# maksimt/rri_nmf

Measured on AMD Instinct MI355X. Metric: RRI sweeps/sec and achieved HBM GB/s on dense X (n x d, rank k), higher is better.
Workload: dtype f64

## Files before the change

### include/rri_hip.h

```cpp
#ifndef RRI_HIP_H
#define RRI_HIP_H

#include <stdint.h>
#include <stddef.h>

#ifdef __cplusplus
extern "C" {
#endif

#define RRI_ABI_VERSION 1
#define RRI_GRAM_SLICES 8
#define RRI_MAX_K 1024

typedef struct rri_ctx rri_ctx;
typedef struct rri_comm rri_comm;
#define RRI_COMM_ID_BYTES 128

typedef int32_t rri_status;
enum {
    RRI_OK = 0,
    RRI_PAUSED = 1,
    RRI_ERR_INVALID = -1,
    RRI_ERR_HIP = -2,
    RRI_ERR_UNSUPPORTED = -3,
// ... 69 lines not shown
rri_status rri_residual_update(rri_ctx* ctx, const double* a, const double* b, const double* a2, const double* b2,
                               const double* trow, const double* wcol, double* y_out, double* z_out);
rri_status rri_get_residual(rri_ctx* ctx, void* host, int64_t ld, int32_t host_dtype);

rri_status rri_project_W_rows(rri_ctx* ctx, double s, const double* s_vec);
rri_status rri_objective(rri_ctx* ctx, double* out);
rri_status rri_argmax_rows(rri_ctx* ctx, int32_t* out_host);
rri_status rri_masked_rmse(rri_ctx* ctx, const int64_t* ij, const double* vals, int64_t count,
                           double clip_lo, double clip_hi, double* out);
rri_status rri_snapshot(rri_ctx* ctx);
rri_status rri_rollback(rri_ctx* ctx);

rri_status rri_X_times(rri_ctx* ctx, const double* B, int32_t m, double* out);
rri_status rri_Xt_times(rri_ctx* ctx, const double* Q, int32_t m, double* out);
rri_status rri_range_finder(rri_ctx* ctx, const double* Q0, int32_t m, int32_t n_iter, int32_t transpose, double* Q_out,
                            double* B_out);
rri_status rri_sparse_range_finder(rri_ctx* ctx, const double* Q0, int32_t m, int32_t n_iter, int32_t transpose, double* Q_out,
                                   double* B_out);

rri_status rri_column_positive_counts(rri_ctx* ctx, double* df_out);
rri_status rri_scale_X(rri_ctx* ctx, const double* col_scale, int32_t normalize_rows);
rri_status rri_csr_column_positive_counts(rri_ctx* ctx, double* df_out);
rri_status rri_csr_scale_X(rri_ctx* ctx, const double* col_scale, int32_t normalize_rows, int64_t* zero_rows_out);

rri_status rri_comm_unique_id(uint8_t* id_out );
rri_status rri_comm_create(rri_comm** out, const uint8_t* id, int32_t rank, int32_t world, int32_t device);
typedef int32_t (*rri_allreduce_fn)(void* user, double* buf, int64_t count);
typedef int32_t (*rri_allgather_fn)(void* user, const double* send, int64_t count, double* recv);
typedef int32_t (*rri_broadcast_fn)(void* user, double* buf, int64_t count, int32_t root);
rri_status rri_comm_create_host(rri_comm** out, int32_t rank, int32_t world, rri_allreduce_fn allreduce,
                                rri_allgather_fn allgather, rri_broadcast_fn broadcast, void* user);
rri_status rri_comm_destroy(rri_comm* comm);
rri_status rri_attach_comm(rri_ctx* ctx, rri_comm* comm, int64_t row_offset, int64_t n_global);
rri_status rri_comm_broadcast(rri_ctx* ctx, double* host, int64_t count, int32_t root);
rri_status rri_comm_allreduce_sum(rri_ctx* ctx, double* host, int64_t count);
rri_status rri_comm_stats(rri_ctx* ctx, int32_t* rank, int32_t* world, int64_t* allreduce_calls);

rri_status rri_reduce_buffer(rri_ctx* ctx, void** dev_ptr, int64_t* n_elems);
rri_status rri_bind_reduce_buffer(rri_ctx* ctx, void* dev_ptr, int64_t n_elems);
rri_status rri_topic_reduce_local(rri_ctx* ctx, int32_t t);
rri_status rri_reduce_read(rri_ctx* ctx, double* out, int64_t count);
rri_status rri_reduce_write(rri_ctx* ctx, const double* in, int64_t count);
rri_status rri_topic_finish(rri_ctx* ctx, int32_t t);
rri_status rri_topic_finish_w(rri_ctx* ctx, int32_t t);
rri_status rri_resid_row_argmax(rri_ctx* ctx, double* value, int64_t* local_row);
rri_status rri_reset_row(rri_ctx* ctx, int64_t local_row, double* row_out_host);
rri_status rri_poll(rri_ctx* ctx);
rri_status rri_objective_parts(rri_ctx* ctx, double out[3]);

rri_status rri_timing_enable(rri_ctx* ctx, int32_t on);
rri_status rri_timing_read(rri_ctx* ctx, int32_t kernel_id, int64_t* launches, double* total_ms);
rri_status rri_synchronize(rri_ctx* ctx);
rri_status rri_onchip_info(rri_ctx* ctx, int32_t* eligible, int64_t* launches);
#define RRI_LAYOUT_FIELDS 19
rri_status rri_layout_info(rri_ctx* ctx, int64_t* out, int32_t n);
rri_status rri_onchip_fallbacks(rri_ctx* ctx, int64_t* fallbacks);
rri_status rri_debug_xcc(rri_ctx* ctx, int32_t* out, int32_t count);
rri_status rri_sweep_until(rri_ctx* ctx, int32_t n_sweeps, double obj_prev, double stop_scale, double* obj_hist,
                           int32_t* sweeps_done);
rri_status rri_bench_rank1_update(rri_ctx* ctx, int32_t reps, double* avg_ms);
rri_status rri_bench_stream_copy(rri_ctx* ctx, int32_t reps, double* avg_ms);

#ifdef __cplusplus
}
#endif
#endif
```

### rri_nmf_amd/_capi.py

```python
import ctypes as C
import os

_PKG = os.path.dirname(os.path.abspath(__file__))
LIB_PATH = os.environ.get('RRI_HIP_LIB', os.path.join(_PKG, 'lib', 'librri_hip.so'))

RRI_GRAM_SLICES = 8
RRI_LAYOUT_FIELDS = 19
RRI_MAX_K = 1024
RRI_OK, RRI_PAUSED = 0, 1
RRI_ERR_INVALID, RRI_ERR_HIP, RRI_ERR_UNSUPPORTED = -1, -2, -3
RRI_ERR_UNBOUNDED, RRI_ERR_W_COL_ZERO, RRI_ERR_NOT_IMPLEMENTED, RRI_ERR_COMM = -4, -5, -6, -7
RRI_COMM_ID_BYTES = 128
RRI_F32, RRI_F64, RRI_F16 = 0, 1, 2
RRI_UNWEIGHTED, RRI_WEIGHTED_DENSE, RRI_WEIGHTED_SPARSE, RRI_UNWEIGHTED_RESIDUAL, RRI_UNWEIGHTED_SPARSE = 0, 1, 2, 3, 4
RESET_NONE, RESET_MAX_RESID_DOCUMENT, RESET_RANDOM = 0, 1, 2
EVENT_NONE, EVENT_RESET_T, EVENT_RESET_W = 0, 1, 2
ABI_VERSION = 1


class Params(C.Structure):
    _fields_ = [('fix_W', C.c_int32), ('fix_T', C.c_int32), ('project_T_each_iter', C.c_int32),
                ('has_t_row_sum', C.c_int32), ('has_w_row_sum', C.c_int32), ('reset_method', C.c_int32),
                ('resets_left', C.c_int32), ('reserved0', C.c_int32),
                ('t_row_sum', C.c_double), ('w_row_sum', C.c_double),
                ('reg_w_l1', C.c_double), ('reg_w_l2', C.c_double), ('reg_t_l1', C.c_double),
                ('reg_t_l2', C.c_double), ('eps_div', C.c_double)]


class Event(C.Structure):
    _fields_ = [('kind', C.c_int32), ('topic', C.c_int32), ('sweep', C.c_int32), ('resume_topic', C.c_int32)]


_P = C.c_void_p
_I32, _I64, _D = C.c_int32, C.c_int64, C.c_double
ALLREDUCE_FN = C.CFUNCTYPE(C.c_int32, C.c_void_p, C.POINTER(C.c_double), C.c_int64)
ALLGATHER_FN = C.CFUNCTYPE(C.c_int32, C.c_void_p, C.POINTER(C.c_double), C.c_int64, C.POINTER(C.c_double))
BROADCAST_FN = C.CFUNCTYPE(C.c_int32, C.c_void_p, C.POINTER(C.c_double), C.c_int64, C.c_int32)
PROTOTYPES = {
    'rri_abi_version': (C.c_uint32, []),
    'rri_create': (_I32, [C.POINTER(_P), _I64, _I64, _I32, _I32, _I32, _I32, _P]),
    'rri_destroy': (_I32, [_P]),
    'rri_last_error': (C.c_char_p, [_P]),
    'rri_upload_X': (_I32, [_P, _P, _I64, _I32]),
    'rri_upload_mask': (_I32, [_P, _P, _I64, _I32]),
    'rri_bind_X_device': (_I32, [_P, _P, _I64]),
    'rri_storage_error': (_I32, [_P, C.POINTER(_D)]),
    'rri_bind_mask_device': (_I32, [_P, _P, _I64]),
    'rri_upload_X_csr': (_I32, [_P, C.POINTER(_I64), C.POINTER(_I32), _P, _I64, _I32]),
    'rri_upload_mask_csr_pattern': (_I32, [_P, C.POINTER(_I64), C.POINTER(_I32), _P, _I64, _I32]),
    'rri_upload_observed_csr': (_I32, [_P, C.POINTER(_I64), C.POINTER(_I32), _P, _I64, _I32]),
    'rri_set_W': (_I32, [_P, _P, _I64, _I32]),
    'rri_set_T': (_I32, [_P, _P, _I64, _I32]),
    'rri_get_W': (_I32, [_P, _P, _I64, _I32]),
    'rri_get_T': (_I32, [_P, _P, _I64, _I32]),
    'rri_set_params': (_I32, [_P, C.POINTER(Params)]),
    'rri_sweep': (_I32, [_P, _I32, C.POINTER(_I32)]),
    'rri_resume': (_I32, [_P, C.POINTER(_I32)]),
    'rri_pending_event': (_I32, [_P, C.POINTER(Event)]),
    'rri_apply_reset_max_resid': (_I32, [_P, _I32, C.POINTER(_I64)]),
    'rri_apply_reset_vectors': (_I32, [_P, _I32, C.POINTER(_D), C.POINTER(_D)]),
# ... 113 lines not shown
```

### rri_nmf_amd/csrc/rri_hip.hip

```cpp
#include <hip/hip_runtime.h>
#include <dlfcn.h>
#include <rccl/rccl.h>

#include <algorithm>
#include <atomic>
#include <chrono>
#include <cstdarg>
#include <cstdio>
#include <mutex>
#include <cstdlib>
#include <cstring>
#include <string>
#include <utility>
#include <vector>

#include "rri_hip.h"
#include "rri_kernels.hpp"
#include "rri_wrri_kernels.hpp"
#include "rri_sparse_kernels.hpp"
#include "rri_onchip_kernels.hpp"

using namespace rri;

namespace {
// ... 39 lines not shown
        a.AllReduce = (decltype(a.AllReduce))dlsym(from, "ncclAllReduce");
        a.AllGather = (decltype(a.AllGather))dlsym(from, "ncclAllGather");
        a.Broadcast = (decltype(a.Broadcast))dlsym(from, "ncclBroadcast");
        a.GetErrorString = (decltype(a.GetErrorString))dlsym(from, "ncclGetErrorString");
        a.CommAbort = (decltype(a.CommAbort))dlsym(from, "ncclCommAbort");
        return a.GetUniqueId && a.CommInitRank && a.CommDestroy && a.AllReduce && a.AllGather && a.Broadcast &&
               a.GetErrorString;
    };
    if (const char* e = getenv("RRI_RCCL_LIB")) {
        h = dlopen(e, RTLD_NOW | RTLD_GLOBAL);
        if (h && resolve(h)) { a.ok = true; return a; }
        a.err = std::string("RRI_RCCL_LIB=") + e + " could not be used";
        return a;
    }
    if (resolve(RTLD_DEFAULT)) { a.ok = true; return a; }
    for (const char* name : {"librccl.so.1", "librccl.so"}) {
        h = dlopen(name, RTLD_NOW | RTLD_GLOBAL);
        if (h && resolve(h)) { a.ok = true; return a; }
    }
    a.err = "RCCL not found (no ncclAllReduce in the process, no librccl.so.1)";
    return a;
}
RcclApi& rccl_api() {
    static RcclApi api = load_rccl();
    return api;
}
}

struct rri_comm {
    int rank = 0, world = 1, device = 0;
    ncclComm_t nccl = nullptr;
    rri_allreduce_fn h_allreduce = nullptr;
    rri_allgather_fn h_allgather = nullptr;
    rri_broadcast_fn h_broadcast = nullptr;
    void* user = nullptr;
    std::vector<double> hbuf, hbuf2;
    long n_allreduce = 0;
    bool aborted = false;
};

constexpr double PASS_CACHE_MB = 256.0;

struct rri_switches {
    bool onchip = true;
    bool onchip_obj = true;
    bool wsweep = true;
    bool obj_direct = false;
    bool wmcorr_cols = true;
    bool wnw_mask = true;
    int pass_rot = -1;
    int rot_cal = 1;
    bool rot_debug = false;
    bool mask_bits = true;
    double pass_cache_mb = PASS_CACHE_MB;
};

struct rri_ctx {
    i64 n = 0, d = 0, LD = 0;
    int k = 0, dtype = RRI_F32, weighted = 0, device = 0;
    size_t es = 4;
    double store_err[2] = {0.0, 0.0};
    int VN = 4, PW = 1024;
    hipStream_t stream = nullptr;
    bool own_stream = false;
    rri_switches sw;

    void *X = nullptr, *M = nullptr, *E = nullptr;
    i64 ldx = 0, ldm = 0;
    bool own_X = false, own_M = false;
    double *W = nullptr, *T = nullptr, *Wprev = nullptr, *Tprev = nullptr;
    double *Ypart = nullptr, *Zpart = nullptr, *red = nullptr, *xraw = nullptr, *Ttpart = nullptr;
    unsigned* Mbits = nullptr;
    i64 ldb = 0;
    double* Qt = nullptr;
    bool q_valid = false;
    int rot_x = 0, rot_r = 0;
    bool rot_done = false;
    int keep_q = -1;
    bool gfull_valid = false;
    double *Gfull = nullptr, *Wsweep0 = nullptr, *wsum_part = nullptr, *wsums = nullptr;
    double *Y2part = nullptr, *Z2part = nullptr, *dtv = nullptr, *dwv = nullptr, *wold = nullptr, *zeros = nullptr;
    i64 ldw = 0;
    int nsplit = 4;
    bool own_red = false;
    i64 red_elems = 0;
    bool sparse = false;
    i64 nnz = 0;
    int sp_max_row = 0, kp = 8;
    i64* sp_rowptr = nullptr;
    int* sp_col = nullptr;
    void *sp_x = nullptr, *sp_e = nullptr;
    double* sp_Tt = nullptr;
    struct SpCopy {
        int nblk = 1, bw = 1, lps = 64, nwork = 0;
        i64 nseg = 0, gdim = 0, count = 0;
        i64* segptr = nullptr;
        unsigned short* idx = nullptr;
        void* val = nullptr;
        int* perm = nullptr;
        SpWork* work = nullptr;
    } sp[2];
    bool sparse_x = false;
    SpWork* spx_work = nullptr;
    double* rowhat = nullptr;
    double* Cpart = nullptr;
    double* N2part = nullptr;
    unsigned* Mcols = nullptr;
    bool nw_mask = false;
    bool mcols_tried = false;
    double mask_density = 1.0;
    int cpart_rows = 0;
    bool wcorr = false;
    int wcorr_topic = 0, wcorr_nrb = 0;
    bool resid_fresh = false;
    bool dt_pending = false;
    bool explicit_resid = false;
    bool dw_pending = false;
    int dw_topic = 0;
    double* told = nullptr;
    double *Gpart = nullptr, *tpart = nullptr, *rowobj = nullptr, *rowpos = nullptr, *normpart = nullptr;
    double *dtmp = nullptr;
    double* objbuf = nullptr;
    i64* itmp = nullptr;
    i64* tpart_idx = nullptr;
    double *resetT = nullptr, *resetW = nullptr;
    DevState* st = nullptr;

    int npanels = 1, rpb = 1, nrb = 1, nwb = 1, ntb = 1;
    int gpart_n = 1;
    int ttpart_n = 0;
    int xy_rows = 0;
    int xy_stride = 1;
    int ntb32 = 1;
    int tpart_n = 1;

    rri_params prm{};
    bool have_params = false, have_X = false, have_W = false, have_T = false, have_M = false;


    bool carry_valid = false;
    int carry_topic = -1;
    double* XYpart = nullptr;
    int xy_run = -1;
    bool xy_valid = false, x_sq_valid = false;
    bool obj_track_pending = false, obj_track_valid = false;
    double obj_track_value = 0.0;
    struct { bool active = false; double prev = 0.0, scale = 0.0; int n = 0; double* out = nullptr; } until;
    double *objhist = nullptr, *objdec = nullptr;
    double x_sq = 0.0;
    bool pending_wcheck = false;
    int pending_wcheck_topic = -1;

    bool paused = false;
    int run_total = 0;
    Cursor resume_at{0, 0, 0};
    bool resume_done = false;
    rri_event pending{RRI_EVENT_NONE, -1, 0, 0};

    bool resid_valid = false;
    bool skip_row_finish = false;
    int nwb256 = 1;

    rri_comm* comm = nullptr;
    i64 row_offset = 0, n_global = 0;
    double* ctail = nullptr;
    double* cand = nullptr;
    rri_status comm_status = RRI_OK;

    int n_cu = 0;
    double *mkZ = nullptr, *mkG = nullptr, *mkP = nullptr, *mkX = nullptr, *mkT = nullptr, *objE = nullptr;
    unsigned* mkbar = nullptr;
    long onchip_launches = 0;
    double *Wsafe = nullptr, *Tsafe = nullptr;
    bool onchip_in_flight = false;
    bool onchip_off = false;
    long long onchip_off_until = 0;
    bool onchip_saved_skip = false;
    long onchip_fallbacks = 0;

    int timing = 0;
    long timing_seq[4] = {0, 0, 0, 0};
    std::vector<TimedLaunch> timed[4];
    std::vector<hipEvent_t> event_pool;
// ... 140 lines not shown
    hipEvent_t e = nullptr;
    (void)hipEventCreate(&e);
    return e;
}
struct TimedScope {
    rri_ctx* c;
    int id;
    TimedLaunch tl{nullptr, nullptr};
    bool on;
    TimedScope(rri_ctx* c_, int id_)
        : c(c_), id(id_),
          on(c_->timing > 0 && (c_->timing_seq[id_]++ % c_->timing) == 0 && c_->timed[id_].size() < 400000) {
        if (on) {
            tl.a = get_event(c);
            tl.b = get_event(c);
            (void)hipEventRecord(tl.a, c->stream);
        }
    }
    ~TimedScope() {
        if (on) {
            (void)hipEventRecord(tl.b, c->stream);
            c->timed[id].push_back(tl);
        }
    }
};

size_t dtype_size(int dt) { return dt == RRI_F32 ? 4 : dt == RRI_F64 ? 8 : dt == RRI_F16 ? 2 : 0; }

void f16_unreachable(rri_ctx* c) {
    if (c->comm_status == RRI_OK) {
        c->comm_status = RRI_ERR_UNSUPPORTED;
        c->err = "this operation rewrites X or needs a mask, a residual or a CSR store: not available on an RRI_F16 handle";
    }
}

template <typename SX>
struct LaunchX {
    typedef SX Elem;
    static constexpr bool RO = std::is_same<SX, _Float16>::value;
    static size_t pass_shmem(const rri_ctx* c, int upd) {
        return ((5 + upd) * (size_t)c->rpb + 4 * 8 * 72) * sizeof(double);
    }
    struct Upd {
        const double *a = nullptr, *b = nullptr, *a2 = nullptr, *b2 = nullptr, *b2sub = nullptr;
    };
    static int stream_whole(const rri_ctx* c) {
        return (double)c->n * (double)c->LD * (double)c->es > 192.0e6 ? 0 : -1;
    }
    template <bool DO_Y, bool DO_Z, int UPD, int U, bool NT, bool RS>
    static void pass_k(rri_ctx* c, void* Xp, i64 ldp, const double* trow, const double* wc, const Upd& u, const TgramJob& job,
                       int keep) {
        const int ncols = (int)std::min<i64>(ldp, c->LD);
        typedef typename std::conditional<(UPD > 0), SX, const SX>::type XT;
        hipLaunchKernelGGL((k_pass<SX, DO_Y, DO_Z, UPD, U, NT, RS>), dim3(c->npanels * c->nrb + job.nblocks), dim3(256),
                           pass_shmem(c, UPD), c->stream, (XT*)Xp, ldp, (int)c->n, ncols, trow, wc, c->Ypart,
                           c->Zpart, c->LD, c->rpb, c->npanels, u.a, u.b, u.a2, u.b2, u.b2sub, (const DevState*)c->st, job,
                           ((ro_pass_interleaved(c) || UPD > 0) ? c->nrb : 0) |
                               ((c->sw.pass_rot >= 0 ? c->sw.pass_rot : (UPD > 0 ? c->rot_r : c->rot_x)) << 27),
                           keep);
    }
    template <bool DO_Y, bool DO_Z, int UPD>
    static void pass_cfg(rri_ctx* c, void* Xp, i64 ldp, const double* trow, const double* wc, int keep, const Upd& u = Upd{},
                         const TgramJob& job = TgramJob{}) {
        constexpr int U = UPD > 0 ? 16 : 8;
        constexpr bool RS = UPD == 0 && DO_Y;
        if (keep >= 0) pass_k<DO_Y, DO_Z, UPD, U, true, RS>(c, Xp, ldp, trow, wc, u, job, keep);
        else pass_k<DO_Y, DO_Z, UPD, U, false, RS>(c, Xp, ldp, trow, wc, u, job, 0);
    }
    template <bool DO_Y, bool DO_Z>
    static void pass(rri_ctx* c, int t, int tz, const TgramJob& job = TgramJob{}) {
        TimedScope ts(c, 0);
        if constexpr (!RO) {
            if (c->sparse_x) {
                spx_pass<DO_Y, DO_Z>(c, c->T + (i64)t * c->LD, c->W + (i64)tz * c->ldw);
                return;
            }
        }
        pass_cfg<DO_Y, DO_Z, 0>(c, c->X, c->ldx, c->T + (i64)t * c->LD, c->W + (i64)tz * c->ldw, c->keep_q, Upd{}, job);
    }
    static void rpass_colsums(rri_ctx* c, int tz) {
        TimedScope ts(c, 0);
        pass_cfg<false, true, 0>(c, c->E, c->LD, nullptr, c->W + (i64)tz * c->ldw, stream_whole(c));
    }
    static void rank_update(rri_ctx* c, void* R, i64 ldr, const Upd& u, const double* trow, const double* wc,
                            const TgramJob& job = TgramJob{}) {
        TimedScope ts(c, 3);
        if (u.a2) pass_cfg<true, true, 2>(c, R, ldr, trow, wc, stream_whole(c), u, job);
        else pass_cfg<true, true, 1>(c, R, ldr, trow, wc, stream_whole(c), u, job);
    }
    template <bool DO_Y, bool DO_Z, bool UPD2, bool WRITE, bool MBITS, int U, bool RS>
    static void wpass_k(rri_ctx* c, const double* trow, const double* wc, const double* a1, const double* b1,
                        const double* a2, const double* b2) {
        if constexpr (DO_Z && MBITS) {
            if (nw_from_mask(c)) { wpass_k2<DO_Y, DO_Z, UPD2, WRITE, MBITS, U, RS, false>(c, trow, wc, a1, b1, a2, b2); return; }
        }
        wpass_k2<DO_Y, DO_Z, UPD2, WRITE, MBITS, U, RS, DO_Z>(c, trow, wc, a1, b1, a2, b2);
    }
    template <bool DO_Y, bool DO_Z, bool UPD2, bool WRITE, bool MBITS, int U, bool RS, bool DO_Z2>
    static void wpass_k2(rri_ctx* c, const double* trow, const double* wc, const double* a1, const double* b1,
                         const double* a2, const double* b2) {
        const int ncols = (int)std::min<i64>(c->ldx, c->LD);
        const int rot = (c->sw.pass_rot >= 0 ? c->sw.pass_rot : c->rot_r) << 27;
        if constexpr (DO_Y && WRITE && U == 4 && (DO_Z2 || !DO_Z)) {
            hipLaunchKernelGGL((k_wpass_occ4<SX, DO_Y, DO_Z, UPD2, WRITE, U, true, MBITS, RS, DO_Z2>), dim3(c->npanels * c->nrb),
                               dim3(256), (11 * (size_t)c->rpb + 4 * 8 * 72) * sizeof(double), c->stream, (SX*)c->E,
                               (const SX*)c->M, c->LD, c->ldm, (const unsigned*)c->Mbits, c->ldb, (int)c->n, ncols, trow,
                               wc, a1, b1, a2, b2, c->Ypart, c->Y2part, c->Zpart, c->Z2part, c->LD, c->rpb, c->npanels,
// ... 368 lines not shown
        }                                       \
    } while (0)
#define DISPATCH_RO(c, expr)                    \
    do {                                        \
        if ((c)->dtype == RRI_F32) {            \
            typedef LaunchX<float> L;           \
            expr;                               \
        } else if ((c)->dtype == RRI_F64) {     \
            typedef LaunchX<double> L;          \
            expr;                               \
        } else {                                \
            typedef LaunchX<_Float16> L;        \
            expr;                               \
        }                                       \
    } while (0)

struct LK {
    static int gpart_rows(const rri_ctx* c) { return c->gpart_n; }
    template <bool UPDATE>
    static void wcol_resid(rri_ctx* c, int t, int tn, int sweep) {
        TimedScope ts(c, 1);
        hipLaunchKernelGGL((k_wcol_resid<UPDATE>), dim3(c->nwb256), dim3(256), 0, c->stream, c->W, c->ldw, (int)c->n,
                           c->k, t, tn, (const double*)c->Ypart, c->npanels, (const double*)c->Ttpart, c->nsplit,
                           c->dwv, c->Gpart, sweep, kparams(c), c->st);
        c->gpart_n = c->nwb256;
    }
    static size_t wcol_shmem(const rri_ctx* c) { return (size_t)(2 * c->k + 2 + 256 + 64) * sizeof(double); }
    template <bool UPDATE, bool CARRY>
    static void wcol_src(rri_ctx* c, int t, int tn, int sweep, const double* ypart, int nslices) {
        TimedScope ts(c, 1);
        hipLaunchKernelGGL((k_wcol<UPDATE, CARRY>), dim3(c->nwb), dim3(256), wcol_shmem(c), c->stream, c->W, c->ldw,
                           (int)c->n, c->k, t, tn, ypart, nslices, (const double*)c->Ttpart, c->ttpart_n, c->Gpart,
                           c->XYpart + (i64)t * c->xy_stride, sweep, kparams(c), c->st);
        c->gpart_n = c->nwb;
        if (UPDATE) note_xy(c, t, c->nwb * WCOL_TILES);
    }
    static void note_xy(rri_ctx* c, int t, int rows) {
        if (t == 0) { c->xy_run = 1; c->xy_rows = rows; }
        else c->xy_run = (c->xy_run == t && c->xy_rows == rows) ? t + 1 : -1;
        c->xy_valid = c->xy_run == c->k;
        c->obj_track_valid = false;
    }
    template <bool UPDATE, bool CARRY>
    static void wcol(rri_ctx* c, int t, int tn, int sweep) {
        wcol_src<UPDATE, CARRY>(c, t, tn, sweep, (const double*)c->Ypart, c->npanels);
    }
    static void reduce(rri_ctx* c) {
        const int nb = (int)((c->LD + 31) / 32) + GRAM_SLICES;
        hipLaunchKernelGGL(k_reduce, dim3(nb), dim3(1024), 0, c->stream, (const double*)c->Zpart, c->LD, c->nrb,
                           (const double*)c->Gpart, gpart_rows(c), c->k, c->red, (const DevState*)c->st);
    }
    static bool light(const rri_ctx* c) { return !(c->prm.project_T_each_iter && c->prm.has_t_row_sum); }
    static void trow(rri_ctx* c, int t, int check_prev, int tprev, int sweep, bool force_final) {
        hipLaunchKernelGGL(k_trow_numer, dim3(c->ntb), dim3(128), 0, c->stream, c->T, c->LD, (int)c->d, c->k, t,
                           (const double*)c->red, c->LD, c->xraw, c->tpart, c->tpart_idx, check_prev, tprev, sweep,
                           kparams(c), c->st, resid_sched(c) ? 1 : 0, resid_sched(c) ? c->told : (double*)nullptr);
        c->tpart_n = c->ntb;
        trow_final_if_needed(c, t, sweep, force_final);
    }
    static bool small(const rri_ctx* c) {
        return (double)gpart_rows(c) * (c->k + 2) * c->ntb32 <= 4.0e6;
    }
    static void trow_small(rri_ctx* c, int t, int check_prev, int tprev, int sweep, bool force_final) {
        hipLaunchKernelGGL(k_trow_small, dim3(c->ntb32), dim3(1024), 0, c->stream, c->T, c->LD, (int)c->d, c->k, t,
                           (const double*)c->Zpart, c->nrb, (const double*)c->Gpart, gpart_rows(c), c->red, c->LD, c->xraw,
                           c->tpart, c->tpart_idx, check_prev, tprev, sweep, kparams(c), c->st, resid_sched(c) ? 1 : 0,
                           resid_sched(c) ? c->told : (double*)nullptr);
        c->tpart_n = c->ntb32;
        trow_final_if_needed(c, t, sweep, force_final);
    }
    static void trow_final_if_needed(rri_ctx* c, int t, int sweep, bool force_final) {
        if (!light(c) || force_final)
            hipLaunchKernelGGL(k_trow_final, dim3(1), dim3(1024), 0, c->stream, c->T, c->LD, (int)c->d, t, c->xraw,
                               (const double*)c->tpart, (const i64*)c->tpart_idx, c->tpart_n, sweep, kparams(c), c->st);
    }
    static void check_prev_only(rri_ctx* c, int tprev, int sweep, int pos) {
        hipLaunchKernelGGL(k_check_red, dim3(1), dim3(64), 0, c->stream, (const double*)c->red, c->LD, c->k, tprev,
                           sweep, pos, kparams(c), c->st);
    }
    static void tgram(rri_ctx* c, int t, int finish, int sweep) {
        c->ttpart_n = c->nsplit;
        hipLaunchKernelGGL(k_tgram, dim3(c->k, c->nsplit), dim3(256), 0, c->stream, (const double*)c->T, c->LD,
                           (int)c->d, c->k, t, c->Ttpart, (const double*)c->tpart, c->tpart_n, finish, sweep,
                           kparams(c), c->st);
    }
    static void scale_wcol(rri_ctx* c, int t) {
        hipLaunchKernelGGL(k_scale_wcol, dim3((unsigned)((c->n + 255) / 256)), dim3(256), 0, c->stream, c->W,
                           c->ldw, (int)c->n, t, (const DevState*)c->st);
    }
    static void check_wcol(rri_ctx* c, int tprev, int sweep, int pos) {
        hipLaunchKernelGGL(k_check_wcol, dim3(1), dim3(256), 0, c->stream, (const double*)c->Gpart, gpart_rows(c), c->k,
                           tprev, sweep, pos, kparams(c), c->st);
    }
    static void proj_rows(rri_ctx* c, double s, const double* svec) {
        hipLaunchKernelGGL(k_proj_rows, dim3((unsigned)((c->n + 255) / 256)), dim3(256), 0, c->stream, c->W, c->ldw, (int)c->n, c->k, s,
                           svec);
    }
    static void norms(rri_ctx* c, const double* A, i64 rows, i64 cols, i64 ld) {
        hipLaunchKernelGGL(k_norms, dim3(256), dim3(256), 0, c->stream, A, rows, cols, ld, c->normpart);
    }
    static void reset_commit(rri_ctx* c, int t) {
        const i64 m = std::max(c->n, c->d);
        hipLaunchKernelGGL(k_reset_commit, dim3((unsigned)((m + 255) / 256)), dim3(256), 0, c->stream, c->W, c->ldw,
                           c->T, c->LD, (int)c->n, (int)c->d, t, (const i64*)c->itmp, (const double*)c->xraw);
    }
    static void set_row_col(rri_ctx* c, int t, const double* trow, const double* wcolv) {
        const i64 m = std::max(c->n, c->d);
        hipLaunchKernelGGL(k_set_row_col, dim3((unsigned)((m + 255) / 256)), dim3(256), 0, c->stream, c->W, c->ldw,
                           c->T, c->LD, (int)c->n, (int)c->d, t, trow, wcolv);
    }
    static void argmax_rows(rri_ctx* c, int* out) {
        hipLaunchKernelGGL(k_argmax_rows, dim3((unsigned)((c->n + 255) / 256)), dim3(256), 0, c->stream,
                           (const double*)c->W, c->ldw, (int)c->n, c->k, out);
    }
    static void masked_sqerr(rri_ctx* c, const i64* ij, const double* vals, i64 count, double lo, double hi) {
        hipLaunchKernelGGL(k_masked_sqerr, dim3(256), dim3(256), 0, c->stream, (const double*)c->W, c->ldw,
                           (const double*)c->T, c->LD, c->k, ij, vals, count, lo, hi, c->normpart);
    }
};

template <typename Src, typename Dst, bool TR>
void launch_convert(rri_ctx* c, const void* src, i64 lds_, void* dst, i64 ldd, i64 rows, i64 cols) {
    const i64 total = rows * cols;
    const unsigned nb = (unsigned)std::min<i64>(4096, (total + 255) / 256);
    hipLaunchKernelGGL((k_convert2d<Src, Dst, TR>), dim3(nb ? nb : 1), dim3(256), 0, c->stream, (const Src*)src,
                       lds_, (Dst*)dst, ldd, rows, cols);
}

rri_status to_device_half(rri_ctx* c, const void* host, i64 ld, int host_dtype, void* dev, i64 ldd, i64 rows, i64 cols,
                          bool transpose) {
    if (transpose) return fail(c, RRI_ERR_INVALID, "float16 storage is for X only");
    const size_t hs = dtype_size(host_dtype);
    const i64 total = rows * cols;
    const unsigned nb = (unsigned)std::max<i64>(1, std::min<i64>(4096, (total + 255) / 256));
    DevTmp tmp, part;
    HIPCHK(c, tmp.alloc((size_t)rows * cols * hs));
    HIPCHK(c, part.alloc((size_t)nb * 3 * sizeof(double)));
// ... 42 lines not shown
        if (transpose) launch_convert<SRC, DST, true>(c, tmp, cols, dev, ldd, rows, cols);  \
        else launch_convert<SRC, DST, false>(c, tmp, cols, dev, ldd, rows, cols);           \
    } while (0)
        if (hf && df) RRI_CONV(float, float);
        else if (hf) RRI_CONV(float, double);
        else if (df) RRI_CONV(double, float);
        else RRI_CONV(double, double);
#undef RRI_CONV
        e = hipStreamSynchronize(c->stream);
    }
    (void)hipFree(tmp);
    if (e != hipSuccess) return fail(c, RRI_ERR_HIP, "upload failed: %s", hipGetErrorString(e));
    return RRI_OK;
}

rri_status to_host(rri_ctx* c, const void* dev, i64 ldd, void* host, i64 ld, int host_dtype, i64 rows, i64 cols,
                   int dev_dtype, bool transpose = false) {
    if (!host || ld < cols) return fail(c, RRI_ERR_INVALID, "bad host matrix (ld=%lld < cols=%lld)", ld, cols);
    if (host_dtype != RRI_F32 && host_dtype != RRI_F64) return fail(c, RRI_ERR_INVALID, "bad host dtype");
    if (dev_dtype != RRI_F32 && dev_dtype != RRI_F64) return fail(c, RRI_ERR_UNSUPPORTED, "nothing stored as float16 is read back");
    const size_t hs = dtype_size(host_dtype);
    const size_t ds = dtype_size(dev_dtype);
    if (host_dtype == dev_dtype && !transpose) {
        HIPCHK(c, hipMemcpy2DAsync(host, ld * hs, dev, ldd * ds, cols * hs, rows, hipMemcpyDeviceToHost,
                                   c->stream));
        HIPCHK(c, hipStreamSynchronize(c->stream));
        return RRI_OK;
    }
    void* tmp = nullptr;
    HIPCHK(c, hipMalloc(&tmp, (size_t)rows * cols * hs));
    {
        const bool hf = host_dtype == RRI_F32, df = dev_dtype == RRI_F32;
#define RRI_CONV(SRC, DST)                                                                     \
    do {                                                                                       \
        if (transpose) launch_convert<SRC, DST, true>(c, dev, ldd, tmp, cols, cols, rows);     \
        else launch_convert<SRC, DST, false>(c, dev, ldd, tmp, cols, rows, cols);              \
    } while (0)
        if (df && hf) RRI_CONV(float, float);
        else if (df) RRI_CONV(float, double);
        else if (hf) RRI_CONV(double, float);
        else RRI_CONV(double, double);
#undef RRI_CONV
    }
    hipError_t e = hipMemcpy2DAsync(host, ld * hs, tmp, cols * hs, cols * hs, rows, hipMemcpyDeviceToHost,
                                    c->stream);
    if (e == hipSuccess) e = hipStreamSynchronize(c->stream);
    (void)hipFree(tmp);
    if (e != hipSuccess) return fail(c, RRI_ERR_HIP, "download failed: %s", hipGetErrorString(e));
    return RRI_OK;
}

void invalidate(rri_ctx* c) {
    c->carry_valid = false;
    c->carry_topic = -1;
    c->resid_valid = false;
    c->xy_run = -1;
    c->xy_valid = false;
    c->obj_track_valid = false;
}

void wcheck_now(rri_ctx* c, int tprev, int sweep, int pos) {
    if (!c->comm) {
        if (c->weighted)
            hipLaunchKernelGGL(k_wcheck_wcol, dim3(1), dim3(256), 0, c->stream, (const double*)c->Gpart, c->nwb256, c->k,
                               tprev, sweep, pos, kparams(c), c->st, (double*)nullptr);
        else LK::check_wcol(c, tprev, sweep, pos);
        return;
    }
    if (c->weighted)
        hipLaunchKernelGGL(k_wcheck_wcol, dim3(1), dim3(256), 0, c->stream, (const double*)c->Gpart, c->nwb256, c->k,
                           tprev, sweep, pos, kparams(c), c->st, c->ctail);
    else
        hipLaunchKernelGGL(k_colsum_tail, dim3(1), dim3(256), 0, c->stream, (const double*)c->Gpart, LK::gpart_rows(c),
                           c->k, c->ctail, (const DevState*)c->st);
    comm_allreduce(c, c->ctail, 2);
    hipLaunchKernelGGL(k_wcheck_tail, dim3(1), dim3(64), 0, c->stream, (const double*)c->ctail, tprev, sweep, pos,
                       kparams(c), c->st);
}

void enqueue_prologue(rri_ctx* c, int t, int sweep) {
    if (c->pending_wcheck) {
        wcheck_now(c, c->pending_wcheck_topic, sweep, t);
        c->pending_wcheck = false;
    }
    LK::wcol<false, true>(c, t, t, sweep);
    DISPATCH_RO(c, (L::template pass<false, true>(c, t, t)));
    c->carry_valid = true;
    c->carry_topic = t;
}

void enqueue_T_half(rri_ctx* c, int sweep, int t, bool standalone) {
    if (!c->carry_valid || c->carry_topic != t) enqueue_prologue(c, t, sweep);
    {
        TimedScope ts(c, 2);
        const int chk = c->pending_wcheck ? 1 : 0;
        if (LK::small(c) && !c->comm) {
            LK::trow_small(c, t, chk, c->pending_wcheck_topic, sweep, standalone);
        } else {
            LK::reduce(c);
            comm_allreduce(c, c->red, c->LD + (i64)GRAM_SLICES * (c->k + 2));
            LK::trow(c, t, chk, c->pending_wcheck_topic, sweep, standalone);
        }
        c->pending_wcheck = false;
        if (c->prm.fix_W && no_regs(c)) LK::scale_wcol(c, t);
    }
    c->carry_valid = false;
    c->resid_valid = false;
    c->q_valid = false; c->gfull_valid = false;
    c->xy_valid = false;
    c->obj_track_valid = false;
}

void enqueue_W_half(rri_ctx* c, int sweep, int t) {
    const int k = c->k;
    const bool carry_next = (k > 1) && !c->prm.fix_T;
    const int tn = (t + 1) % k;
    const int finish = (LK::light(c) && !c->prm.fix_T && !c->skip_row_finish) ? 1 : 0;
    c->skip_row_finish = false;
    TgramJob job{};
    if (c->prm.fix_T || c->sparse_x) {
        TimedScope ts(c, 2);
        LK::tgram(c, t, finish, sweep);
    } else {
        job = TgramJob{(const double*)c->T, c->LD, (int)c->d, c->k, t, c->Ttpart, (const double*)c->tpart, c->tpart_n,
                       c->nsplit, finish, sweep, kparams(c), c->st, c->k * c->nsplit};
        c->ttpart_n = c->nsplit;
    }
    if (carry_next) {
        DISPATCH_RO(c, (L::template pass<true, true>(c, t, tn, job)));
        LK::wcol<true, true>(c, t, tn, sweep);
        c->carry_valid = true;
        c->carry_topic = tn;
        c->pending_wcheck = true;
        c->pending_wcheck_topic = t;
    } else {
        if (c->prm.fix_T) {
            if (!c->q_valid) {
                DISPATCH_RO(c, L::xtt(c));
                c->q_valid = true;
            }
            LK::wcol_src<true, false>(c, t, tn, sweep, c->Qt + (i64)t * c->ldw, 1);
        } else {
            DISPATCH_RO(c, (L::template pass<true, false>(c, t, tn, job)));
            LK::wcol<true, false>(c, t, tn, sweep);
        }
        int ns = sweep, np = t + 1;
        if (np == k) { np = 0; ns = sweep + 1; }
        wcheck_now(c, t, ns, np);
        c->carry_valid = false;
    }
    c->resid_valid = false;
}

void r_refresh(rri_ctx* c) {
    DISPATCH(c, L::resid(c, false, true, nullptr, nullptr));
    c->resid_valid = true;
    c->resid_fresh = true;
    c->dw_pending = false;
    c->dt_pending = false;
}

void enqueue_rT_half(rri_ctx* c, int sweep, int t, bool standalone) {
    if (!c->resid_valid) r_refresh(c);
    if (!c->carry_valid || c->carry_topic != t) {
        if (c->pending_wcheck) {
            wcheck_now(c, c->pending_wcheck_topic, sweep, t);
            c->pending_wcheck = false;
        }
        if (c->dw_pending) r_refresh(c);
        LK::wcol_resid<false>(c, t, t, sweep);
        DISPATCH(c, L::rpass_colsums(c, t));
        c->carry_valid = true;
        c->carry_topic = t;
    }
    {
        TimedScope ts(c, 2);
        const int chk = c->pending_wcheck ? 1 : 0;
        if (LK::small(c) && !c->comm) {
            LK::trow_small(c, t, chk, c->pending_wcheck_topic, sweep, standalone);
        } else {
            LK::reduce(c);
            comm_allreduce(c, c->red, c->LD + (i64)GRAM_SLICES * (c->k + 2));
            LK::trow(c, t, chk, c->pending_wcheck_topic, sweep, standalone);
        }
        c->pending_wcheck = false;
    }
    c->carry_valid = false;
    c->resid_fresh = false;
    c->dt_pending = true;
    c->xy_valid = false;
    c->obj_track_valid = false;
}

void enqueue_rW_half(rri_ctx* c, int sweep, int t) {
    const int k = c->k;
    const int tn = (t + 1) % k;
    if (!c->resid_valid) r_refresh(c);
    const int finish = (LK::light(c) && !c->skip_row_finish) ? 1 : 0;
    c->skip_row_finish = false;
    const TgramJob job{(const double*)c->T, c->LD, (int)c->d, c->k, t, c->Ttpart, (const double*)c->tpart, c->tpart_n,
                       c->nsplit, finish, sweep, kparams(c), c->st, c->k * c->nsplit};
    c->ttpart_n = c->nsplit;
    const double* trow = c->T + (i64)t * c->LD;
    DISPATCH(c, {
        typename L::Upd u;
        u.a = c->dw_pending ? c->dwv : c->zeros;
        u.b = c->T + (i64)(c->dw_pending ? c->dw_topic : t) * c->LD;
        u.a2 = c->W + (i64)t * c->ldw;
        u.b2 = trow;
        u.b2sub = c->dt_pending ? c->told : trow;
        L::rank_update(c, c->E, c->LD, u, trow, c->W + (i64)tn * c->ldw, job);
    });
    LK::wcol_resid<true>(c, t, tn, sweep);
    c->dw_pending = true;
    c->dw_topic = t;
    c->dt_pending = false;
    c->resid_fresh = false;
    c->carry_valid = true;
    c->carry_topic = tn;
    c->pending_wcheck = true;
    c->pending_wcheck_topic = t;
}

void w_refresh(rri_ctx* c) {
    DISPATCH(c, L::resid(c, true, true, nullptr, nullptr));
    c->resid_valid = true;
    c->resid_fresh = true;
    c->dt_pending = false;
    c->dw_pending = false;
    c->carry_valid = false;
}

void w_reduce(rri_ctx* c, bool take_check = false, int sweep = 0, int pos = 0) {
    const int nb = (int)((c->LD + 63) / 64);
    const int chk = (take_check && c->pending_wcheck) ? 1 : 0;
    const bool nwm = c->nw_mask;
    hipLaunchKernelGGL(k_wreduce, dim3(nb), dim3(1024), 0, c->stream, (const double*)c->Zpart,
                       (const double*)(nwm ? c->N2part : c->Z2part), c->LD, c->nrb, nwm ? c->wcorr_nrb : c->nrb, c->wcorr ? (const double*)c->Cpart : (const double*)nullptr, c->wcorr_nrb,
                       (const double*)(c->T + (i64)c->wcorr_topic * c->LD), c->red, (const double*)c->Gpart, c->nwb256, c->k, chk,
                       c->pending_wcheck_topic, sweep, pos, kparams(c), c->st);
    if (chk) c->pending_wcheck = false;
}

bool wtrow_small(const rri_ctx* c) { return !c->comm && c->nrb <= 64; }

void enqueue_wT_sums(rri_ctx* c, int t, bool fused = false, bool take_check = false, int sweep = 0) {
    const double* wt_t = c->W + (i64)t * c->ldw;
    if (!c->carry_valid || c->carry_topic != t)
        DISPATCH(c, (L::template wpass<false, true, false, false>(c, nullptr, wt_t, c->zeros, c->zeros, nullptr, nullptr)));
    c->wcorr = !c->sparse && c->dw_pending;
    c->nw_mask = false;
    DISPATCH(c, c->nw_mask = L::nw_from_mask(c));
    if (c->wcorr || c->nw_mask) {
        if (c->wcorr) c->wcorr_topic = c->dw_topic;
        DISPATCH(c, L::wmcorr(c, wt_t, c->wcorr ? c->dwv : nullptr));
// ... 405 lines not shown
                                                "closed form", "-", "slices arrive", "-", "project", "-"};
                for (int w = 0; w < 2; ++w) {
                    fprintf(stderr, "rri on-chip sections, workgroup %s (us total):", w == 0 ? "0 (worker)" : "G-1");
                    for (int i = 0; i < 13; ++i) fprintf(stderr, " %s %.1f;", names[i], h[16 * w + i] * 0.01);
                    fprintf(stderr, "\n");
                }
            }
            (void)hipMemsetAsync(dbg, 0, 32 * sizeof(long long), c->stream);
            a.dbg = dbg;
        }
    }
    (void)hipMemcpyAsync(c->Wsafe, c->W, (size_t)k * c->ldw * 8, hipMemcpyDeviceToDevice, c->stream);
    (void)hipMemcpyAsync(c->Tsafe, c->T, (size_t)k * c->LD * 8, hipMemcpyDeviceToDevice, c->stream);
    c->onchip_saved_skip = c->skip_row_finish;
    hipError_t e;
    {
        TimedLaunch tl{nullptr, nullptr};
        const bool timed = c->timing > 0 && c->timed[0].size() < 400000;
        if (timed) { tl.a = get_event(c); tl.b = get_event(c); (void)hipEventRecord(tl.a, c->stream); }
        const bool proj = !LK::light(c);
        if (c->k > ONCHIP_SMALL_K) {
            if (c->dtype == RRI_F64) {
                if (proj) e = g.rpw <= 4 ? onchip_launch<double, 4, false, true, 8>(c, g, a) : onchip_launch<double, ONCHIP_MAX_RPW_K64_PROJ / 2, false, true, 8>(c, g, a);
                else e = g.rpw <= 4 ? onchip_launch<double, 4, false, false, 8>(c, g, a) : onchip_launch<double, ONCHIP_MAX_RPW_K64 / 2, false, false, 8>(c, g, a);
            } else if (proj) e = g.rpw <= 8 ? onchip_launch<float, 8, false, true, 8>(c, g, a) : onchip_launch<float, ONCHIP_MAX_RPW_K64_PROJ, false, true, 8>(c, g, a);
            else e = g.rpw <= 8 ? onchip_launch<float, 8, false, false, 8>(c, g, a) : onchip_launch<float, ONCHIP_MAX_RPW_K64, false, false, 8>(c, g, a);
        } else if (c->dtype == RRI_F64) {
            if (proj) e = g.rpw <= 4 ? onchip_launch<double, 4, false, true>(c, g, a) : onchip_launch<double, ONCHIP_MAX_RPW / 2, false, true>(c, g, a);
            else e = g.rpw <= 4 ? onchip_launch<double, 4>(c, g, a) : onchip_launch<double, ONCHIP_MAX_RPW / 2>(c, g, a);
        } else if (proj && a.dbg) e = g.rpw <= 8 ? onchip_launch<float, 8, true, true>(c, g, a) : onchip_launch<float, ONCHIP_MAX_RPW, true, true>(c, g, a);
        else if (proj) e = g.rpw <= 8 ? onchip_launch<float, 8, false, true>(c, g, a) : onchip_launch<float, ONCHIP_MAX_RPW, false, true>(c, g, a);
        else if (a.dbg) e = g.rpw <= 8 ? onchip_launch<float, 8, true>(c, g, a) : onchip_launch<float, ONCHIP_MAX_RPW, true>(c, g, a);
        else if (g.rpw <= 8) e = onchip_launch<float, 8>(c, g, a);
        else e = onchip_launch<float, ONCHIP_MAX_RPW>(c, g, a);
        if (timed) { (void)hipEventRecord(tl.b, c->stream); c->timed[0].push_back(tl); }
    }
    if (e != hipSuccess) {
        if (getenv("RRI_ONCHIP_DEBUG")) fprintf(stderr, "rri: on-chip sweep not launched (%s): rows/wg %d, rows/wave %d, LDS %zu B\n", hipGetErrorString(e), g.rows_wg, g.rpw, g.shmem);
        (void)hipGetLastError();
        return false;
    }
    c->onchip_launches += 1;
    c->onchip_in_flight = true;
    if (const char* path = getenv("RRI_ONCHIP_LOG")) {
        if (FILE* f = fopen(path, "a")) {
            fprintf(f, "%lld %lld %d %s %s sweeps %d..%d\n", (long long)c->n, (long long)c->d, k, c->dtype == RRI_F32 ? "f32" : "f64",
                    LK::light(c) ? "plain" : "simplex", cur.sweep, c->run_total);
            fclose(f);
        }
    }
    const bool whole_last = c->run_total - 1 > cur.sweep || (cur.topic == 0 && cur.phase == 0);
    c->carry_valid = false; c->carry_topic = -1;
    c->pending_wcheck = false;
    c->resid_valid = false; c->q_valid = false; c->gfull_valid = false;
    c->skip_row_finish = false;
    c->xy_run = whole_last ? k : -1;
    c->xy_rows = g.G;
    c->xy_valid = whole_last;
    c->obj_track_valid = false;
    c->obj_track_pending = a.track != 0;
    return true;
}

void enqueue_final_check(rri_ctx* c, int sweep_arg) {
    if (c->pending_wcheck) {
        wcheck_now(c, c->pending_wcheck_topic, sweep_arg, 0);
        c->pending_wcheck = false;
    }
}

void enqueue_from(rri_ctx* c, Cursor cur) {
    if (cur.sweep < c->run_total && onchip_ok(c) && enqueue_onchip(c, cur)) return;
    if (c->until.active && cur.sweep < c->run_total) c->run_total = cur.sweep + 1;
    enqueue_range(c, cur, c->run_total);
    enqueue_final_check(c, c->run_total);
}

rri_status read_state(rri_ctx* c, DevState* out) {
    HIPCHK(c, hipMemcpyAsync(out, c->st, sizeof(DevState), hipMemcpyDeviceToHost, c->stream));
    HIPCHK(c, hipStreamSynchronize(c->stream));
    if (c->comm_status != RRI_OK) {
        const rri_status r = c->comm_status;
        c->comm_status = RRI_OK;
        invalidate(c);
        c->pending_wcheck = false;
        return r;
    }
    return RRI_OK;
}

rri_status status_from_halt(rri_ctx* c, const DevState& s, int32_t* sweeps_done) {
    if (s.halt == 0) {
        c->paused = false;
        if (sweeps_done) *sweeps_done = c->run_total;
        return RRI_OK;
    }
    invalidate(c);
    c->pending_wcheck = false;
    if (s.halt == HALT_EVENT_STOP) {
        c->paused = false;
        if (sweeps_done) *sweeps_done = s.halt_sweep;
        return RRI_OK;
    }
    if (s.halt > 0) {
        if (c->until.active) c->run_total = std::min(c->run_total, (s.halt == HALT_EVENT_RESET_W && s.halt_pos == 0) ? s.halt_sweep : s.halt_sweep + 1);
        c->paused = true;
        c->pending.kind = s.halt == HALT_EVENT_RESET_T ? RRI_EVENT_RESET_T : RRI_EVENT_RESET_W;
        c->pending.topic = s.halt_topic;
        c->pending.sweep = s.halt_sweep;
        c->pending.resume_topic = s.halt_pos;
        if (s.halt == HALT_EVENT_RESET_T) c->resume_at = Cursor{s.halt_sweep, s.halt_topic, 1};
        else c->resume_at = Cursor{s.halt_sweep, s.halt_pos, 0};
        if (sweeps_done) *sweeps_done = s.halt_sweep;
        return RRI_PAUSED;
    }
    c->paused = false;
    if (sweeps_done) *sweeps_done = s.halt_sweep;
    switch (s.halt) {
        case HALT_ERR_UNBOUNDED:
            return fail(c, RRI_ERR_UNBOUNDED, "Minimum objective is unbounded (topic %d)", s.halt_topic);
        case HALT_ERR_W_COL_ZERO:
            return fail(c, RRI_ERR_W_COL_ZERO, "W[:, t] sums to 0 (topic %d)", s.halt_topic);
        case HALT_ERR_NOT_IMPLEMENTED:
            return fail(c, RRI_ERR_NOT_IMPLEMENTED, "s=%g is not yet implemented", c->prm.t_row_sum);
        case HALT_ERR_GRID_SYNC:
            return fail(c, RRI_ERR_HIP, "the persistent sweep's workgroups could not synchronise (not all resident); RRI_ONCHIP=0 selects the launch-per-phase schedule");
        default:
            return fail(c, RRI_ERR_INVALID, "unknown device status %d", s.halt);
    }
}

rri_status clear_halt(rri_ctx* c) {
    HIPCHK(c, hipMemsetAsync(c->st, 0, 32, c->stream));
    return RRI_OK;
}

int pass_keep(const rri_ctx* c) {
    const double chain = 8.0 * ((double)c->k * (double)c->ldw + 2.0 * (double)c->nrb * (double)c->LD +
                                2.0 * (double)c->npanels * (double)c->n + 2.0 * (double)c->k * (double)c->LD +
                                2.0 * (double)c->nwb * (double)(c->k + 2));
    const double budget = c->sw.pass_cache_mb * 1.0e6 - chain;
    const double block = (double)c->rpb * (double)c->LD * (double)c->es;
    if ((double)c->n * (double)c->LD * (double)c->es <= budget) return -1;
    return budget > 0.0 ? (int)std::min((double)c->nrb, std::floor(budget / block)) : 0;
}

rri_switches read_switches() {
    rri_switches sw;
    if (const char* e = getenv("RRI_ONCHIP")) sw.onchip = atoi(e) != 0;
    if (const char* e = getenv("RRI_ONCHIP_OBJ")) sw.onchip_obj = atoi(e) != 0;
    if (const char* e = getenv("RRI_WSWEEP")) sw.wsweep = atoi(e) != 0;
    if (const char* e = getenv("RRI_OBJ_DIRECT")) sw.obj_direct = atoi(e) != 0;
    if (const char* e = getenv("RRI_WMCORR_COLS")) sw.wmcorr_cols = atoi(e) != 0;
    if (const char* e = getenv("RRI_WNW_MASK")) sw.wnw_mask = atoi(e) != 0;
    if (const char* e = getenv("RRI_PASS_ROT")) sw.pass_rot = atoi(e) & 7;
    if (const char* e = getenv("RRI_ROT_CAL")) sw.rot_cal = std::max(0, atoi(e));
    sw.rot_debug = getenv("RRI_ROT_DEBUG") != nullptr;
    if (const char* e = getenv("RRI_MASK_BITS")) sw.mask_bits = atoi(e) != 0;
    if (const char* e = getenv("RRI_PASS_CACHE_MB")) sw.pass_cache_mb = std::max(0.0, atof(e));
    return sw;
}

const char* sparse_data_refusal(const rri_ctx* c) {
    return c->sparse_x ? "an RRI_UNWEIGHTED_SPARSE handle keeps X as CSR: it takes its data through rri_upload_X_csr only "
                         "(no dense X, no device binding, no mask)"
                       : "a sparse-pattern handle takes its data through rri_upload_observed_csr";
}

#define REFUSE_F16(c, what)                                                                                             \
    if ((c)->dtype == RRI_F16)                                                                                          \
        return fail((c), RRI_ERR_UNSUPPORTED, "%s is not available on an RRI_F16 handle (float16 stores a dense X that is only read)", what)

rri_status ready(rri_ctx* c) {
    if (!c->have_X || !c->have_W || !c->have_T || !c->have_params)
        return fail(c, RRI_ERR_INVALID, "X, W, T and params must be set before stepping");
    if (c->weighted && !c->have_M) return fail(c, RRI_ERR_INVALID, "weighted handle without a mask");
    return RRI_OK;
}

}

extern "C" {

uint32_t rri_abi_version(void) { return RRI_ABI_VERSION; }

const char* rri_last_error(const rri_ctx* ctx) { return ctx ? ctx->err.c_str() : g_create_error.c_str(); }

rri_status rri_create(rri_ctx** out, int64_t n, int64_t d, int32_t k, int32_t dtype, int32_t weighted,
                      int32_t device, void* stream) {
    if (!out) return RRI_ERR_INVALID;
    *out = nullptr;
    if (n < 1 || d < 1 || k < 1) return fail(nullptr, RRI_ERR_INVALID, "need n,d,k >= 1 (got %lld,%lld,%d)", n, d, k);
    if (dtype != RRI_F32 && dtype != RRI_F64 && dtype != RRI_F16) return fail(nullptr, RRI_ERR_INVALID, "dtype must be RRI_F32, RRI_F64 or RRI_F16");
    if (n > 2000000000LL || d > 2000000000LL) return fail(nullptr, RRI_ERR_INVALID, "n, d must fit int32");
    if (k > RRI_MAX_K) return fail(nullptr, RRI_ERR_UNSUPPORTED, "k=%d is above the rank limit RRI_MAX_K = %d of the device path", k, RRI_MAX_K);
    int ndev = 0;
    if (hipGetDeviceCount(&ndev) != hipSuccess || ndev < 1)
        return fail(nullptr, RRI_ERR_HIP, "no HIP device available (librri_hip needs an MI355X)");
    if (device < 0 || device >= ndev) return fail(nullptr, RRI_ERR_INVALID, "device %d out of range [0,%d)", device, ndev);
    if (weighted < 0 || weighted > 4)
        return fail(nullptr, RRI_ERR_INVALID, "weighted must be RRI_UNWEIGHTED, RRI_WEIGHTED_DENSE, RRI_WEIGHTED_SPARSE, "
                                              "RRI_UNWEIGHTED_RESIDUAL or RRI_UNWEIGHTED_SPARSE");
    if (dtype == RRI_F16 && weighted != RRI_UNWEIGHTED) {
        static const char* const flavour[] = {"", "RRI_WEIGHTED_DENSE", "RRI_WEIGHTED_SPARSE", "RRI_UNWEIGHTED_RESIDUAL", "RRI_UNWEIGHTED_SPARSE"};
        const bool rewritten = weighted == RRI_WEIGHTED_DENSE || weighted == RRI_UNWEIGHTED_RESIDUAL;
        return fail(nullptr, RRI_ERR_UNSUPPORTED, "RRI_F16 stores a read-only dense X (RRI_UNWEIGHTED); %s %s", flavour[weighted],
                    rewritten ? "rewrites its stored residual at every topic step, which float16 would round every time"
                              : "keeps its values in a CSR store, which has no float16 layout");
    }
    rri_ctx* c = new rri_ctx();
    const bool explicit_resid = weighted == RRI_UNWEIGHTED_RESIDUAL;
// ... 35 lines not shown
            const i64 r = (n + nrb_t - 1) / nrb_t;
            if (r >= rows_min || total == 512) rpb = r;
        }
    }
    rpb = std::max<i64>(rpb, 32);
    rpb = std::min<i64>(round_up(rpb, 16), rpb_cap);
    c->rpb = (int)rpb;
    c->nrb = (int)((n + rpb - 1) / rpb);
    if (c->sparse) {
        const i64 block_bytes = SP_BLOCK_BYTES;
        const i64 cap = sparse_x ? std::min<i64>(spx_block_cap(), std::max<i64>(64, (block_bytes / 8 - 64) / 64 * 64))
                                 : block_bytes / (3 * (i64)c->es);
        for (int w = 0; w < 2; ++w) {
            rri_ctx::SpCopy& cp = c->sp[w];
            cp.gdim = w == 0 ? d : n;
            cp.nseg = w == 0 ? n : d;
            cp.nblk = (int)((cp.gdim + cap - 1) / cap);
            cp.bw = (int)round_up((cp.gdim + cp.nblk - 1) / cp.nblk, 64);
        }
        c->npanels = c->sp[0].nblk;
        c->nrb = c->sp[1].nblk;
    }
    c->nwb = (int)((n + 64 * WCOL_TILES - 1) / (64 * WCOL_TILES));
    c->nwb256 = (int)((n + 255) / 256);
    c->ldw = n;
    c->keep_q = pass_keep(c);
    c->ntb = (int)((d + 127) / 128);
    c->ntb32 = (int)((c->LD + 31) / 32);
    c->tpart_n = c->ntb;
    c->nsplit = (int)std::max<i64>(1, std::min<i64>(8, d / 2048));
    c->red_elems = round_up(std::max<i64>(c->LD + (i64)GRAM_SLICES * (k + 2), weighted ? 2 * c->LD + 2 : 0), 4);

    const size_t f8 = sizeof(double);
    const size_t es_x = c->es;
    CR(hipMalloc((void**)&c->W, (size_t)k * c->ldw * f8));
    CR(hipMalloc((void**)&c->T, (size_t)k * c->LD * f8));
    CR(hipMemsetAsync(c->T, 0, (size_t)k * c->LD * f8, c->stream));
    CR(hipMalloc((void**)&c->Ypart, (size_t)c->npanels * n * f8));
    CR(hipMemsetAsync(c->Ypart, 0, (size_t)c->npanels * n * f8, c->stream));
    CR(hipMalloc((void**)&c->Zpart, (size_t)c->nrb * c->LD * f8));
    CR(hipMemsetAsync(c->Zpart, 0, (size_t)c->nrb * c->LD * f8, c->stream));
    const size_t grows = (size_t)std::max(c->nwb, c->nrb);
    c->gpart_n = c->nwb;
    c->xy_stride = (int)std::max<size_t>(std::max<size_t>(grows, (size_t)c->nwb * WCOL_TILES), (size_t)std::max(c->n_cu, 1));
    CR(hipMalloc((void**)&c->Gpart, grows * (k + 2) * sizeof(double)));
    CR(hipMemsetAsync(c->Gpart, 0, grows * (k + 2) * sizeof(double), c->stream));
    CR(hipMalloc((void**)&c->XYpart, (size_t)k * c->xy_stride * f8));
    CR(hipMemsetAsync(c->XYpart, 0, (size_t)k * c->xy_stride * f8, c->stream));
    CR(hipMalloc((void**)&c->red, (size_t)c->red_elems * f8));
    CR(hipMemsetAsync(c->red, 0, (size_t)c->red_elems * f8, c->stream));
    c->own_red = true;
    CR(hipMalloc((void**)&c->xraw, (size_t)c->LD * f8));
    CR(hipMemsetAsync(c->xraw, 0, (size_t)c->LD * f8, c->stream));
    const size_t ttn = (size_t)std::max(c->nsplit, c->ntb32);
    c->ttpart_n = c->nsplit;
    CR(hipMalloc((void**)&c->Ttpart, ttn * k * f8));
    CR(hipMemsetAsync(c->Ttpart, 0, ttn * k * f8, c->stream));
    CR(hipMalloc((void**)&c->Qt, (size_t)k * c->ldw * f8));
    const size_t ntp = (size_t)std::max(c->ntb, c->ntb32);
    CR(hipMalloc((void**)&c->tpart, ntp * sizeof(double)));
    CR(hipMemsetAsync(c->tpart, 0, ntp * sizeof(double), c->stream));
    CR(hipMalloc((void**)&c->tpart_idx, ntp * sizeof(i64)));
    CR(hipMalloc((void**)&c->normpart, 256 * 3 * sizeof(double)));
    CR(hipMalloc((void**)&c->objbuf, (size_t)(2 * k * k + k) * sizeof(double)));
    CR(hipMalloc((void**)&c->dtmp, 16 * sizeof(double)));
    CR(hipMalloc((void**)&c->itmp, 16 * sizeof(i64)));
    if (weighted) {
        const i64 zn = std::max<i64>(c->LD, n);
        if (!c->sparse) {
            CR(hipMalloc(&c->E, (size_t)n * c->LD * es_x));
            if (c->LD != d) CR(hipMemsetAsync(c->E, 0, (size_t)n * c->LD * es_x, c->stream));
        }
        CR(hipMalloc((void**)&c->Y2part, (size_t)c->npanels * n * f8));
        CR(hipMemsetAsync(c->Y2part, 0, (size_t)c->npanels * n * f8, c->stream));
        CR(hipMalloc((void**)&c->Z2part, (size_t)c->nrb * c->LD * f8));
        CR(hipMemsetAsync(c->Z2part, 0, (size_t)c->nrb * c->LD * f8, c->stream));
        if (!c->sparse) {
            c->cpart_rows = (int)std::max<i64>(256, (n + 2047) / 2048);
            CR(hipMalloc((void**)&c->Cpart, (size_t)c->cpart_rows * c->LD * f8));
            CR(hipMemsetAsync(c->Cpart, 0, (size_t)c->cpart_rows * c->LD * f8, c->stream));
            CR(hipMalloc((void**)&c->N2part, (size_t)c->cpart_rows * c->LD * f8));
            CR(hipMemsetAsync(c->N2part, 0, (size_t)c->cpart_rows * c->LD * f8, c->stream));
        }
        CR(hipMalloc((void**)&c->dtv, (size_t)c->LD * f8));
        CR(hipMalloc((void**)&c->dwv, (size_t)n * f8));
        CR(hipMalloc((void**)&c->wold, (size_t)n * f8));
        CR(hipMalloc((void**)&c->zeros, (size_t)zn * f8));
        CR(hipMemsetAsync(c->zeros, 0, (size_t)zn * f8, c->stream));
        CR(hipMemsetAsync(c->dtv, 0, (size_t)c->LD * f8, c->stream));
        if (c->sparse) {
            CR(hipMalloc((void**)&c->sp_Tt, (size_t)d * c->kp * f8));
            CR(hipMemsetAsync(c->sp_Tt, 0, (size_t)d * c->kp * f8, c->stream));
        }
    }
    if (sparse_x) {
        CR(hipMalloc((void**)&c->sp_Tt, (size_t)d * c->kp * f8));
        CR(hipMemsetAsync(c->sp_Tt, 0, (size_t)d * c->kp * f8, c->stream));
    }
    if (explicit_resid) {
        const i64 zn = std::max<i64>(c->LD, n);
        CR(hipMalloc(&c->E, (size_t)n * c->LD * es_x));
        if (c->LD != d) CR(hipMemsetAsync(c->E, 0, (size_t)n * c->LD * es_x, c->stream));
        CR(hipMalloc((void**)&c->dwv, (size_t)n * f8));
        CR(hipMemsetAsync(c->dwv, 0, (size_t)n * f8, c->stream));
        CR(hipMalloc((void**)&c->told, (size_t)c->LD * f8));
        CR(hipMemsetAsync(c->told, 0, (size_t)c->LD * f8, c->stream));
        CR(hipMalloc((void**)&c->zeros, (size_t)zn * f8));
        CR(hipMemsetAsync(c->zeros, 0, (size_t)zn * f8, c->stream));
    }
    CR(hipMalloc((void**)&c->st, sizeof(DevState)));
    CR(hipMemsetAsync(c->st, 0, sizeof(DevState), c->stream));
    if (dtype == RRI_F32) CR(LaunchX<float>::set_attrs());
    else if (dtype == RRI_F64) CR(LaunchX<double>::set_attrs());
    else CR(LaunchX<_Float16>::set_attrs());
    CR(hipStreamSynchronize(c->stream));
#undef CR
    *out = c;
    return RRI_OK;
}

rri_status rri_destroy(rri_ctx* c) {
    if (!c) return RRI_OK;
    (void)hipSetDevice(c->device);
    if (c->stream) (void)hipStreamSynchronize(c->stream);
    if (c->own_X) (void)hipFree(c->X);
    if (c->own_M) (void)hipFree(c->M);
    void* bufs[] = {c->E, (void*)c->W, (void*)c->T, (void*)c->Wprev, (void*)c->Tprev,                     (void*)c->Ypart, (void*)c->Zpart, (void*)c->xraw, (void*)c->Ttpart, (void*)c->Gpart,
                    (void*)c->tpart, (void*)c->tpart_idx, (void*)c->rowobj, (void*)c->rowpos, (void*)c->normpart,
                    (void*)c->dtmp, (void*)c->itmp, (void*)c->resetT, (void*)c->resetW, (void*)c->st, (void*)c->Y2part,
                    (void*)c->Z2part, (void*)c->Mbits, (void*)c->Qt, (void*)c->dtv, (void*)c->dwv, (void*)c->wold, (void*)c->zeros,
                    (void*)c->XYpart, (void*)c->objbuf, (void*)c->told, (void*)c->Cpart, (void*)c->N2part, (void*)c->Mcols, (void*)c->Gfull, (void*)c->Wsweep0, (void*)c->wsum_part, (void*)c->wsums, (void*)c->ctail, (void*)c->cand, (void*)c->mkZ, (void*)c->mkG, (void*)c->mkP, (void*)c->mkX, (void*)c->mkT, (void*)c->objE, (void*)c->objhist, (void*)c->objdec, (void*)c->mkbar, (void*)c->Wsafe, (void*)c->Tsafe, (void*)c->sp_rowptr, (void*)c->sp_col, c->sp_x, c->sp_e, (void*)c->sp_Tt, (void*)c->spx_work, (void*)c->rowhat,
                    (void*)c->sp[0].segptr, (void*)c->sp[0].idx, c->sp[0].val, (void*)c->sp[0].perm, (void*)c->sp[0].work,
                    (void*)c->sp[1].segptr, (void*)c->sp[1].idx, c->sp[1].val, (void*)c->sp[1].perm, (void*)c->sp[1].work};
    for (void* b : bufs)
        if (b) (void)hipFree(b);
    if (c->own_red && c->red) (void)hipFree(c->red);
    for (int i = 0; i < 4; ++i)
        for (auto& tl : c->timed[i]) { (void)hipEventDestroy(tl.a); (void)hipEventDestroy(tl.b); }
    for (auto e : c->event_pool) (void)hipEventDestroy(e);
    if (c->own_stream && c->stream) (void)hipStreamDestroy(c->stream);
    delete c;
    return RRI_OK;
}

rri_status rri_upload_X(rri_ctx* c, const void* host, int64_t ld, int32_t host_dtype) {
    CHECK_CTX(c);
    if (c->sparse) return fail(c, RRI_ERR_UNSUPPORTED, "%s", sparse_data_refusal(c));
    HIPCHK(c, hipSetDevice(c->device));
    if (c->X && !c->own_X) c->X = nullptr;
    if (!c->X) {
        HIPCHK(c, hipMalloc(&c->X, (size_t)c->n * c->LD * c->es));
        c->own_X = true;
        if (c->LD != c->d) HIPCHK(c, hipMemsetAsync(c->X, 0, (size_t)c->n * c->LD * c->es, c->stream));
    }
    c->ldx = c->LD;
    c->store_err[0] = c->store_err[1] = 0.0;
    rri_status s = to_device(c, host, ld, host_dtype, c->X, c->ldx, c->n, c->d, c->dtype);
    if (s == RRI_OK || c->dtype == RRI_F16) { c->have_X = s == RRI_OK; invalidate(c); c->q_valid = false; c->gfull_valid = false; c->x_sq_valid = false; }
    return s;
}

rri_status rri_upload_mask(rri_ctx* c, const void* host, int64_t ld, int32_t host_dtype) {
    CHECK_CTX(c);
    REFUSE_F16(c, "a mask");
    if (c->sparse) return fail(c, RRI_ERR_UNSUPPORTED, "%s", sparse_data_refusal(c));
    if (!c->weighted) return fail(c, RRI_ERR_INVALID, "handle was not created with weighted=1");
    HIPCHK(c, hipSetDevice(c->device));
    if (c->M && !c->own_M) c->M = nullptr;
    if (!c->M) {
        HIPCHK(c, hipMalloc(&c->M, (size_t)c->n * c->LD * c->es));
        c->own_M = true;
        if (c->LD != c->d) HIPCHK(c, hipMemsetAsync(c->M, 0, (size_t)c->n * c->LD * c->es, c->stream));
    }
    c->ldm = c->LD;
    rri_status s = to_device(c, host, ld, host_dtype, c->M, c->ldm, c->n, c->d, c->dtype);
    if (s == RRI_OK) {
        c->have_M = true;
        invalidate(c);
        DISPATCH(c, s = L::pack_mask_if_binary(c));
        if (s != RRI_OK) return fail(c, s, "packing the mask failed");
        if (c->Mbits && c->own_M) { (void)hipFree(c->M); c->M = nullptr; c->own_M = false; }
    }
    return s;
}

namespace {
struct CsrDev {
    i64* indptr = nullptr;
    int* indices = nullptr;
    void* data = nullptr;
    ~CsrDev() { (void)hipFree(indptr); (void)hipFree(indices); (void)hipFree(data); }
};
rri_status csr_to_device(rri_ctx* c, const int64_t* indptr, const int32_t* indices, const void* data, int64_t nnz,
                         int32_t data_dtype, CsrDev& out) {
    if (!indptr || (nnz > 0 && (!indices || !data)) || nnz < 0) return fail(c, RRI_ERR_INVALID, "bad CSR arrays");
    if (data_dtype != RRI_F32 && data_dtype != RRI_F64) return fail(c, RRI_ERR_INVALID, "bad CSR data dtype");
    if (indptr[0] != 0 || indptr[c->n] != nnz) return fail(c, RRI_ERR_INVALID, "indptr does not span nnz");
    for (i64 r = 0; r < c->n; ++r)
        if (indptr[r + 1] < indptr[r]) return fail(c, RRI_ERR_INVALID, "indptr not monotone at row %lld", r);
    for (i64 p = 0; p < nnz; ++p)
        if (indices[p] < 0 || indices[p] >= c->d) return fail(c, RRI_ERR_INVALID, "column index out of range at %lld", p);
    const size_t ds = dtype_size(data_dtype);
    HIPCHK(c, hipMalloc((void**)&out.indptr, (size_t)(c->n + 1) * sizeof(i64)));
    HIPCHK(c, hipMalloc((void**)&out.indices, (size_t)std::max<i64>(nnz, 1) * sizeof(int)));
    HIPCHK(c, hipMalloc(&out.data, (size_t)std::max<i64>(nnz, 1) * ds));
    HIPCHK(c, hipMemcpyAsync(out.indptr, indptr, (size_t)(c->n + 1) * sizeof(i64), hipMemcpyHostToDevice, c->stream));
    if (nnz > 0) {
        HIPCHK(c, hipMemcpyAsync(out.indices, indices, (size_t)nnz * sizeof(int), hipMemcpyHostToDevice, c->stream));
        HIPCHK(c, hipMemcpyAsync(out.data, data, (size_t)nnz * ds, hipMemcpyHostToDevice, c->stream));
    }
    return RRI_OK;
}
}

static rri_status upload_X_csr_kept(rri_ctx* c, const int64_t* indptr, const int32_t* indices, const void* data,
                                    int64_t nnz, int32_t data_dtype);

rri_status rri_upload_X_csr(rri_ctx* c, const int64_t* indptr, const int32_t* indices, const void* data,
                            int64_t nnz, int32_t data_dtype) {
    CHECK_CTX(c);
    REFUSE_F16(c, "X from CSR arrays");
    if (c->sparse_x) return upload_X_csr_kept(c, indptr, indices, data, nnz, data_dtype);
    if (c->sparse) return fail(c, RRI_ERR_UNSUPPORTED, "%s", sparse_data_refusal(c));
    HIPCHK(c, hipSetDevice(c->device));
    CsrDev dv;
    rri_status s = csr_to_device(c, indptr, indices, data, nnz, data_dtype, dv);
    if (s != RRI_OK) return s;
    if (c->X && !c->own_X) c->X = nullptr;
    if (!c->X) {
        HIPCHK(c, hipMalloc(&c->X, (size_t)c->n * c->LD * c->es));
        c->own_X = true;
    }
    c->ldx = c->LD;
    HIPCHK(c, hipMemsetAsync(c->X, 0, (size_t)c->n * c->LD * c->es, c->stream));
    const unsigned nb = (unsigned)((c->n + 3) / 4);
    if (c->dtype == RRI_F32) {
        if (data_dtype == RRI_F32) hipLaunchKernelGGL((k_csr_scatter<float, float>), dim3(nb), dim3(256), 0, c->stream, dv.indptr, dv.indices, (const float*)dv.data, c->n, (float*)c->X, c->ldx);
        else hipLaunchKernelGGL((k_csr_scatter<double, float>), dim3(nb), dim3(256), 0, c->stream, dv.indptr, dv.indices, (const double*)dv.data, c->n, (float*)c->X, c->ldx);
    } else {
        if (data_dtype == RRI_F32) hipLaunchKernelGGL((k_csr_scatter<float, double>), dim3(nb), dim3(256), 0, c->stream, dv.indptr, dv.indices, (const float*)dv.data, c->n, (double*)c->X, c->ldx);
        else hipLaunchKernelGGL((k_csr_scatter<double, double>), dim3(nb), dim3(256), 0, c->stream, dv.indptr, dv.indices, (const double*)dv.data, c->n, (double*)c->X, c->ldx);
    }
    HIPCHK(c, hipStreamSynchronize(c->stream));
    c->have_X = true;
    invalidate(c);
    c->q_valid = false; c->gfull_valid = false;
    c->x_sq_valid = false;
    return RRI_OK;
}

namespace {
rri_status build_sp_store(rri_ctx* c, const int64_t* indptr, const int32_t* indices, int64_t nnz, int32_t data_dtype,
                          CsrDev& dv, int target_items);
}
static rri_status upload_X_csr_kept(rri_ctx* c, const int64_t* indptr, const int32_t* indices, const void* data,
                                    int64_t nnz, int32_t data_dtype) {
    if (nnz >= 2147483647LL) return fail(c, RRI_ERR_UNSUPPORTED, "more than 2^31-1 stored entries");
    if (!indptr || (nnz > 0 && (!indices || !data)) || nnz < 0) return fail(c, RRI_ERR_INVALID, "bad CSR arrays");
    if (data_dtype != RRI_F32 && data_dtype != RRI_F64) return fail(c, RRI_ERR_INVALID, "bad CSR data dtype");
    if (indptr[0] != 0 || indptr[c->n] != nnz) return fail(c, RRI_ERR_INVALID, "indptr does not span nnz");
    for (i64 r = 0; r < c->n; ++r)
        if (indptr[r + 1] < indptr[r]) return fail(c, RRI_ERR_INVALID, "indptr not monotone at row %lld", r);
    HIPCHK(c, hipSetDevice(c->device));
    const size_t ds = dtype_size(data_dtype);
    std::vector<int32_t> sidx;
    std::vector<unsigned char> sval;
    for (i64 r = 0; r < c->n; ++r) {
        bool sorted = true;
        for (i64 p = indptr[r] + 1; p < indptr[r + 1] && sorted; ++p) sorted = indices[p] > indices[p - 1];
        if (sorted) continue;
        if (sidx.empty()) {
            sidx.assign(indices, indices + nnz);
            sval.assign((const unsigned char*)data, (const unsigned char*)data + (size_t)nnz * ds);
        }
        std::vector<i64> ord((size_t)(indptr[r + 1] - indptr[r]));
        for (size_t q = 0; q < ord.size(); ++q) ord[q] = indptr[r] + (i64)q;
        std::stable_sort(ord.begin(), ord.end(), [&](i64 a, i64 b) { return indices[a] < indices[b]; });
        for (size_t q = 0; q < ord.size(); ++q) {
            sidx[(size_t)indptr[r] + q] = indices[ord[q]];
            std::memcpy(sval.data() + ((size_t)indptr[r] + q) * ds, (const unsigned char*)data + (size_t)ord[q] * ds, ds);
        }
    }
    if (!sidx.empty()) { indices = sidx.data(); data = sval.data(); }
    for (i64 r = 0; r < c->n; ++r)
        for (i64 p = indptr[r] + 1; p < indptr[r + 1]; ++p)
            if (indices[p] == indices[p - 1])
                return fail(c, RRI_ERR_INVALID, "row %lld stores column %d twice (sum the duplicates first)", r, indices[p]);
    CsrDev dv;
    rri_status s = csr_to_device(c, indptr, indices, data, nnz, data_dtype, dv);
    if (s != RRI_OK) return s;
    const int target_items = std::max(1, c->n_cu / 2);
    s = build_sp_store(c, indptr, indices, nnz, data_dtype, dv, target_items);
    if (s != RRI_OK) return s;
    if (nnz > 0)
        DISPATCH(c, for (int w = 0; w < 2; ++w)
                        hipLaunchKernelGGL((k_sp_permute<typename L::Elem>), dim3(2048), dim3(256), 0, c->stream,
                                           (const typename L::Elem*)c->sp_x, (const int*)c->sp[w].perm, c->sp[w].count,
                                           (typename L::Elem*)c->sp[w].val));
    if (c->spx_work) { (void)hipFree(c->spx_work); c->spx_work = nullptr; }
    const int nw0 = c->sp[0].nwork, nw1 = c->sp[1].nwork;
    HIPCHK(c, hipMalloc((void**)&c->spx_work, (size_t)std::max(1, nw0 + nw1) * sizeof(SpWork)));
    if (nw0 > 0) HIPCHK(c, hipMemcpyAsync(c->spx_work, c->sp[0].work, (size_t)nw0 * sizeof(SpWork), hipMemcpyDeviceToDevice, c->stream));
    if (nw1 > 0) HIPCHK(c, hipMemcpyAsync(c->spx_work + nw0, c->sp[1].work, (size_t)nw1 * sizeof(SpWork), hipMemcpyDeviceToDevice, c->stream));
    HIPCHK(c, hipStreamSynchronize(c->stream));
    c->have_X = true;
    invalidate(c);
    c->q_valid = false; c->gfull_valid = false;
    c->x_sq_valid = false;
    return RRI_OK;
}

rri_status rri_upload_mask_csr_pattern(rri_ctx* c, const int64_t* indptr, const int32_t* indices, const void* data,
                                       int64_t nnz, int32_t data_dtype) {
    CHECK_CTX(c);
    REFUSE_F16(c, "a mask");
    if (c->sparse) return fail(c, RRI_ERR_UNSUPPORTED, "%s", sparse_data_refusal(c));
    if (!c->weighted) return fail(c, RRI_ERR_INVALID, "handle was not created with weighted=1");
    HIPCHK(c, hipSetDevice(c->device));
    CsrDev dv;
    rri_status s = csr_to_device(c, indptr, indices, data, nnz, data_dtype, dv);
    if (s != RRI_OK) return s;
    if (c->M && c->own_M) (void)hipFree(c->M);
    c->M = nullptr;
    c->own_M = false;
    c->ldm = c->LD;
    if (c->Mbits) { (void)hipFree(c->Mbits); c->Mbits = nullptr; }
    if (c->Mcols) { (void)hipFree(c->Mcols); c->Mcols = nullptr; }
    c->mcols_tried = false;
    c->ldb = (c->LD + 3) / 4;
    const size_t words = (size_t)((c->n + 7) / 8) * c->ldb;
    HIPCHK(c, hipMalloc((void**)&c->Mbits, words * sizeof(unsigned)));
    HIPCHK(c, hipMemsetAsync(c->Mbits, 0, words * sizeof(unsigned), c->stream));
    const unsigned nb = (unsigned)((c->n + 3) / 4);
    if (data_dtype == RRI_F32) hipLaunchKernelGGL((k_csr_pattern_bits<float>), dim3(nb), dim3(256), 0, c->stream, dv.indptr, dv.indices, (const float*)dv.data, c->n, c->Mbits, c->ldb);
    else hipLaunchKernelGGL((k_csr_pattern_bits<double>), dim3(nb), dim3(256), 0, c->stream, dv.indptr, dv.indices, (const double*)dv.data, c->n, c->Mbits, c->ldb);
    HIPCHK(c, hipStreamSynchronize(c->stream));
    c->have_M = true;
    invalidate(c);
    return RRI_OK;
}

namespace {
rri_status build_sp_store(rri_ctx* c, const int64_t* indptr, const int32_t* indices, int64_t nnz, int32_t data_dtype,
                          CsrDev& dv, int target_items) {
    i64 longest_row = 0;
    for (i64 r = 0; r < c->n; ++r) longest_row = std::max<i64>(longest_row, (i64)(indptr[r + 1] - indptr[r]));
    void* old[] = {(void*)c->sp_rowptr, (void*)c->sp_col, c->sp_x, c->sp_e};
    for (void* b : old)
        if (b) (void)hipFree(b);
    c->sp_rowptr = dv.indptr; dv.indptr = nullptr;
    c->sp_col = dv.indices; dv.indices = nullptr;
    c->sp_x = nullptr; c->sp_e = nullptr;
    const size_t cnt = (size_t)std::max<i64>(nnz, 1);
    HIPCHK(c, hipMalloc(&c->sp_x, cnt * c->es));
    if (nnz > 0) {
        const bool hf = data_dtype == RRI_F32, df = c->dtype == RRI_F32;
        if (hf && df) launch_convert<float, float, false>(c, dv.data, nnz, c->sp_x, nnz, 1, nnz);
        else if (hf) launch_convert<float, double, false>(c, dv.data, nnz, c->sp_x, nnz, 1, nnz);
        else if (df) launch_convert<double, float, false>(c, dv.data, nnz, c->sp_x, nnz, 1, nnz);
        else launch_convert<double, double, false>(c, dv.data, nnz, c->sp_x, nnz, 1, nnz);
// ... 87 lines not shown
    c->nnz = nnz;
    c->sp_max_row = (int)longest_row;
    return RRI_OK;
}
}

rri_status rri_upload_observed_csr(rri_ctx* c, const int64_t* indptr, const int32_t* indices, const void* values,
                                   int64_t nnz, int32_t data_dtype) {
    CHECK_CTX(c);
    REFUSE_F16(c, "an observation pattern");
    if (!c->sparse || c->sparse_x) return fail(c, RRI_ERR_INVALID, "handle was not created with weighted=RRI_WEIGHTED_SPARSE");
    if (nnz >= 2147483647LL) return fail(c, RRI_ERR_UNSUPPORTED, "more than 2^31-1 observed entries");
    HIPCHK(c, hipSetDevice(c->device));
    CsrDev dv;
    rri_status s = csr_to_device(c, indptr, indices, values, nnz, data_dtype, dv);
    if (s != RRI_OK) return s;
    for (i64 r = 0; r < c->n; ++r)
        for (i64 p = indptr[r] + 1; p < indptr[r + 1]; ++p)
            if (indices[p] <= indices[p - 1])
                return fail(c, RRI_ERR_INVALID, "column indices of row %lld are not strictly increasing", r);
    const int target_items = std::max(1, c->n_cu);
    s = build_sp_store(c, indptr, indices, nnz, data_dtype, dv, target_items);
    if (s != RRI_OK) return s;
    HIPCHK(c, hipMalloc(&c->sp_e, (size_t)std::max<i64>(nnz, 1) * c->es));
    c->have_X = true;
    c->have_M = true;
    invalidate(c);
    return RRI_OK;
}

rri_status rri_storage_error(rri_ctx* c, double out[2]) {
    CHECK_CTX(c);
    if (!out) return fail(c, RRI_ERR_INVALID, "out is NULL");
    out[0] = c->store_err[0];
    out[1] = c->store_err[1];
    return RRI_OK;
}

rri_status rri_bind_X_device(rri_ctx* c, const void* dev, int64_t ld) {
    CHECK_CTX(c);
    if (c->sparse) return fail(c, RRI_ERR_UNSUPPORTED, "%s", sparse_data_refusal(c));
    if (!dev || ld < c->d || (ld * (i64)c->es) % 16 || ((uintptr_t)dev) % 16)
        return fail(c, RRI_ERR_INVALID, "device X must be 16-byte aligned with a 16-byte-multiple row stride >= d");
    if (c->d % c->VN) return fail(c, RRI_ERR_INVALID, "binding device X needs d %% %d == 0 (no pad columns)", c->VN);
    HIPCHK(c, hipSetDevice(c->device));
    HIPCHK(c, hipDeviceSynchronize());
    if (c->X && c->own_X) (void)hipFree(c->X);
    c->X = const_cast<void*>(dev);
    c->own_X = false;
    c->ldx = ld;
    c->store_err[0] = c->store_err[1] = 0.0;
    c->have_X = true;
    invalidate(c);
    c->q_valid = false; c->gfull_valid = false;
    c->x_sq_valid = false;
    return RRI_OK;
}

rri_status rri_bind_mask_device(rri_ctx* c, const void* dev, int64_t ld) {
    CHECK_CTX(c);
    REFUSE_F16(c, "a mask");
    if (c->sparse) return fail(c, RRI_ERR_UNSUPPORTED, "%s", sparse_data_refusal(c));
    if (!c->weighted) return fail(c, RRI_ERR_INVALID, "handle was not created with weighted=1");
    if (!dev || ld < c->d || (ld * (i64)c->es) % 16 || ((uintptr_t)dev) % 16)
        return fail(c, RRI_ERR_INVALID, "device mask must be 16-byte aligned with a 16-byte-multiple row stride >= d");
    if (c->d % c->VN) return fail(c, RRI_ERR_INVALID, "binding a device mask needs d %% %d == 0", c->VN);
    HIPCHK(c, hipSetDevice(c->device));
    HIPCHK(c, hipDeviceSynchronize());
    if (c->M && c->own_M) (void)hipFree(c->M);
    c->M = const_cast<void*>(dev);
    c->own_M = false;
    c->ldm = ld;
    c->have_M = true;
    invalidate(c);
    rri_status ps = RRI_OK;
    DISPATCH(c, ps = L::pack_mask_if_binary(c));
    if (ps != RRI_OK) return fail(c, ps, "packing the mask failed");
    return RRI_OK;
}

rri_status rri_set_W(rri_ctx* c, const void* host, int64_t ld, int32_t host_dtype) {
    CHECK_CTX(c);
    HIPCHK(c, hipSetDevice(c->device));
    rri_status s = to_device(c, host, ld, host_dtype, c->W, c->ldw, c->n, c->k, RRI_F64, true);
    if (s == RRI_OK) { c->have_W = true; invalidate(c); c->pending_wcheck = false; }
    return s;
}
rri_status rri_set_T(rri_ctx* c, const void* host, int64_t ld, int32_t host_dtype) {
    CHECK_CTX(c);
    HIPCHK(c, hipSetDevice(c->device));
    rri_status s = to_device(c, host, ld, host_dtype, c->T, c->LD, c->k, c->d, RRI_F64);
    if (s == RRI_OK) { c->have_T = true; invalidate(c); c->q_valid = false; c->gfull_valid = false; }
    return s;
}
rri_status rri_get_W(rri_ctx* c, void* host, int64_t ld, int32_t host_dtype) {
    CHECK_CTX(c);
    HIPCHK(c, hipSetDevice(c->device));
    return to_host(c, c->W, c->ldw, host, ld, host_dtype, c->n, c->k, RRI_F64, true);
}
rri_status rri_get_T(rri_ctx* c, void* host, int64_t ld, int32_t host_dtype) {
    CHECK_CTX(c);
    HIPCHK(c, hipSetDevice(c->device));
    return to_host(c, c->T, c->LD, host, ld, host_dtype, c->k, c->d, RRI_F64);
}

rri_status rri_set_params(rri_ctx* c, const rri_params* p) {
    CHECK_CTX(c);
    if (!p) return fail(c, RRI_ERR_INVALID, "params is NULL");
    if (p->has_t_row_sum && !(p->t_row_sum > 0)) return fail(c, RRI_ERR_INVALID, "t_row_sum must be > 0");
    if (p->has_w_row_sum && !(p->w_row_sum > 0)) return fail(c, RRI_ERR_INVALID, "w_row_sum must be > 0");
    if (p->reset_method < 0 || p->reset_method > 2) return fail(c, RRI_ERR_INVALID, "bad reset_method");
    if (p->fix_W && p->fix_T) return fail(c, RRI_ERR_INVALID, "fix_W and fix_T together leave nothing to update");
    const bool form_before = c->have_params && resid_sched(c);
    if (c->have_params && (c->prm.reg_w_l1 != p->reg_w_l1 || c->prm.reg_w_l2 != p->reg_w_l2 || c->prm.reg_t_l1 != p->reg_t_l1 ||
                           c->prm.reg_t_l2 != p->reg_t_l2))
        c->obj_track_valid = false;
    c->prm = *p;
    c->have_params = true;
    if (c->explicit_resid && form_before != resid_sched(c)) {
        invalidate(c);
        c->dw_pending = false;
        c->dt_pending = false;
    }
    return RRI_OK;
}

static rri_status run_and_collect(rri_ctx* c, Cursor from, int32_t* sweeps_done) {
    HIPCHK(c, hipSetDevice(c->device));
    c->onchip_in_flight = false;
    c->obj_track_pending = false;
    enqueue_from(c, from);
    hipError_t le = hipGetLastError();
    if (le != hipSuccess) return fail(c, RRI_ERR_HIP, "kernel launch failed: %s", hipGetErrorString(le));
    DevState s;
    rri_status r = read_state(c, &s);
    if (r != RRI_OK) return r;
    if (c->onchip_in_flight && s.halt == HALT_ERR_GRID_SYNC) {
        c->onchip_in_flight = false;
        c->onchip_fallbacks += 1;
        c->onchip_off = true;
        c->onchip_off_until = steady_now_ns() + (2000000000LL << std::min<long>(c->onchip_fallbacks - 1, 5));
        long long backoff_ms = 2000;
        if (const char* e = getenv("RRI_ONCHIP_BACKOFF_MS")) backoff_ms = std::max(0, atoi(e));
        g_onchip_backoff_until.store(steady_now_ns() + backoff_ms * 1000000LL);
        if (getenv("RRI_ONCHIP_DEBUG")) fprintf(stderr, "rri: the persistent sweep gave up; sweeps %d.. rerun launch by launch\n", from.sweep);
// ... 44 lines not shown
    if (r != RRI_OK || !c->until.out) return r;
    const int done = sweeps_done ? std::min(std::max(*sweeps_done, 0), c->until.n) : 0;
    for (int i = 0; i < c->until.n; ++i) c->until.out[i] = std::nan("");
    if (done > 0 && c->objhist && c->onchip_launches > 0) {
        hipError_t e = hipMemcpyAsync(c->until.out, c->objhist, (size_t)done * 8, hipMemcpyDeviceToHost, c->stream);
        if (e == hipSuccess) e = hipStreamSynchronize(c->stream);
        if (e != hipSuccess) return fail(c, RRI_ERR_HIP, "objective history: %s", hipGetErrorString(e));
    }
    return r;
}

rri_status rri_sweep_until(rri_ctx* c, int32_t n_sweeps, double obj_prev, double stop_scale, double* obj_hist, int32_t* sweeps_done) {
    CHECK_CTX(c);
    rri_status r = ready(c);
    if (r != RRI_OK) return r;
    if (c->paused) return fail(c, RRI_ERR_INVALID, "a paused run is pending: resolve the event and call rri_resume");
    if (n_sweeps < 1 || !obj_hist || !sweeps_done) return fail(c, RRI_ERR_INVALID, "n_sweeps < 1, or no place for the history / the count");
    HIPCHK(c, hipSetDevice(c->device));
    if (!onchip_ok(c) || n_sweeps > ONCHIP_UNTIL_CAP || !c->sw.onchip_obj)
        return fail(c, RRI_ERR_UNSUPPORTED, "rri_sweep_until needs the register-resident sweep (rri_onchip_info) and at most %d sweeps", ONCHIP_UNTIL_CAP);
    r = ensure_x_sq(c);
    if (r != RRI_OK) return r;
    if (c->objhist) HIPCHK(c, hipMemsetAsync(c->objhist, 0xFF, (size_t)n_sweeps * 8, c->stream));
    c->until.active = true; c->until.prev = obj_prev; c->until.scale = stop_scale; c->until.n = n_sweeps; c->until.out = obj_hist;
    c->run_total = n_sweeps;
    r = clear_halt(c);
    if (r != RRI_OK) { c->until.active = false; return r; }
    r = run_and_collect(c, Cursor{0, 0, 0}, sweeps_done);
    if (r != RRI_OK && r != RRI_PAUSED) c->until.active = false;
    return until_finish(c, r, sweeps_done);
}

rri_status rri_resume(rri_ctx* c, int32_t* sweeps_done) {
    CHECK_CTX(c);
    if (!c->paused) return fail(c, RRI_ERR_INVALID, "nothing to resume");
    if (c->pending.kind != RRI_EVENT_NONE) return fail(c, RRI_ERR_INVALID, "pending event not resolved");
    c->paused = false;
    rri_status r = clear_halt(c);
    if (r != RRI_OK) return r;
    int32_t done_local = 0;
    r = run_and_collect(c, c->resume_at, sweeps_done ? sweeps_done : &done_local);
    if (r != RRI_OK && r != RRI_PAUSED) c->until.active = false;
    return until_finish(c, r, sweeps_done ? sweeps_done : &done_local);
}

rri_status rri_pending_event(rri_ctx* c, rri_event* ev) {
    CHECK_CTX(c);
    if (!ev) return fail(c, RRI_ERR_INVALID, "ev is NULL");
    *ev = c->paused ? c->pending : rri_event{RRI_EVENT_NONE, -1, 0, 0};
    return RRI_OK;
}

static void event_resolved(rri_ctx* c) {
    c->q_valid = false; c->gfull_valid = false;
    if (c->pending.kind == RRI_EVENT_RESET_T) c->skip_row_finish = true;
    c->pending.kind = RRI_EVENT_NONE;
    if (c->prm.resets_left > 0) c->prm.resets_left -= 1;
    invalidate(c);
}

rri_status rri_apply_reset_max_resid(rri_ctx* c, int32_t t, int64_t* row_chosen) {
    CHECK_CTX(c);
    if (t < 0 || t >= c->k) return fail(c, RRI_ERR_INVALID, "topic out of range");
    HIPCHK(c, hipSetDevice(c->device));
    if (!c->rowpos) HIPCHK(c, hipMalloc((void**)&c->rowpos, (size_t)c->n * sizeof(double)));
    HIPCHK(c, clear_halt(c) == RRI_OK ? hipSuccess : hipErrorUnknown);
    DISPATCH_RO(c, L::resid(c, false, false, nullptr, c->rowpos));
    hipLaunchKernelGGL(k_vec_sum_argmax, dim3(1), dim3(1024), 0, c->stream, (const double*)c->rowpos, c->n,
                       (double*)nullptr, c->itmp);
    if (c->comm) {
        rri_comm* m = c->comm;
        hipLaunchKernelGGL(k_pack_candidate, dim3(1), dim3(1), 0, c->stream, (const double*)c->rowpos,
                           (const i64*)c->itmp, c->row_offset, c->ctail);
        comm_allgather(c, c->ctail, 2, c->cand);
        std::vector<double> cand((size_t)2 * m->world);
        hipError_t he = hipMemcpyAsync(cand.data(), c->cand, cand.size() * 8, hipMemcpyDeviceToHost, c->stream);
        if (he == hipSuccess) he = hipStreamSynchronize(c->stream);
        if (he != hipSuccess) return comm_abort(c, "reading the reset candidates", he);
        int win = 0;
        for (int r = 1; r < m->world; ++r)
            if (cand[2 * r] > cand[2 * win] || (cand[2 * r] == cand[2 * win] && cand[2 * r + 1] < cand[2 * win + 1])) win = r;
        if (m->rank == win) DISPATCH_RO(c, L::reset_row(c));
        comm_broadcast(c, c->xraw, c->LD, win);
        if (m->rank != win) {
            const i64 none = -1;
            HIPCHK(c, hipMemcpyAsync(c->itmp, &none, sizeof(i64), hipMemcpyHostToDevice, c->stream));
        }
        LK::reset_commit(c, t);
        HIPCHK(c, hipStreamSynchronize(c->stream));
        if (c->comm_status != RRI_OK) { const rri_status r = c->comm_status; c->comm_status = RRI_OK; return r; }
        if (row_chosen) *row_chosen = (int64_t)cand[2 * win + 1];
        if (c->paused && c->pending.kind != RRI_EVENT_NONE) event_resolved(c);
        else invalidate(c);
        return RRI_OK;
    }
    DISPATCH_RO(c, L::reset_row(c));
    LK::reset_commit(c, t);
    i64 mi = -1;
    HIPCHK(c, hipMemcpyAsync(&mi, c->itmp, sizeof(i64), hipMemcpyDeviceToHost, c->stream));
    HIPCHK(c, hipStreamSynchronize(c->stream));
    if (row_chosen) *row_chosen = mi;
    if (c->paused && c->pending.kind != RRI_EVENT_NONE) event_resolved(c);
    else invalidate(c);
    return RRI_OK;
}

rri_status rri_apply_reset_vectors(rri_ctx* c, int32_t t, const double* T_row, const double* W_col) {
// ... 261 lines not shown
    HIPCHK(c, hipSetDevice(c->device));
    double s = 0.0;
    hipError_t e = hipSuccess;
    if (count > 0 && !bad) {
        i64* dij = nullptr;
        double* dv = nullptr;
        e = hipMalloc((void**)&dij, (size_t)count * 2 * sizeof(i64));
        if (e == hipSuccess) e = hipMalloc((void**)&dv, (size_t)count * sizeof(double));
        if (e == hipSuccess) e = hipMemcpyAsync(dij, ij, (size_t)count * 2 * sizeof(i64), hipMemcpyHostToDevice, c->stream);
        if (e == hipSuccess) e = hipMemcpyAsync(dv, vals, (size_t)count * sizeof(double), hipMemcpyHostToDevice, c->stream);
        double h[256];
        if (e == hipSuccess) {
            LK::masked_sqerr(c, dij, dv, count, lo, hi);
            e = hipMemcpyAsync(h, c->normpart, sizeof h, hipMemcpyDeviceToHost, c->stream);
        }
        if (e == hipSuccess) e = hipStreamSynchronize(c->stream);
        if (dij) (void)hipFree(dij);
        if (dv) (void)hipFree(dv);
        if (e == hipSuccess)
            for (int b = 0; b < 256; ++b) s += h[b];
    }
    double tot[4] = {bad ? 0.0 : s, bad ? 0.0 : (double)count, bad ? 1.0 : 0.0, e != hipSuccess ? 1.0 : 0.0};
    if (c->comm) {
        const rri_status r = comm_allreduce_host(c, tot, 4);
        if (r != RRI_OK) return r;
    }
    if (bad) return bad_entry >= 0 ? fail(c, RRI_ERR_INVALID, "entry %lld out of range", bad_entry) : fail(c, RRI_ERR_INVALID, "%s", bad);
    if (e != hipSuccess) return fail(c, RRI_ERR_HIP, "masked rmse failed: %s", hipGetErrorString(e));
    if (tot[2] > 0.0) return fail(c, RRI_ERR_INVALID, "bad entry list on another rank (%d of them)", (int)tot[2]);
    if (tot[3] > 0.0) return fail(c, RRI_ERR_HIP, "masked rmse failed on another rank");
    if (!(tot[1] > 0.0)) return fail(c, RRI_ERR_INVALID, "no entry on any rank");
    *out = std::sqrt(tot[0] / tot[1]);
    return RRI_OK;
}

rri_status rri_snapshot(rri_ctx* c) {
    CHECK_CTX(c);
    HIPCHK(c, hipSetDevice(c->device));
    if (!c->Wprev) HIPCHK(c, hipMalloc((void**)&c->Wprev, (size_t)c->k * c->ldw * 8));
    if (!c->Tprev) HIPCHK(c, hipMalloc((void**)&c->Tprev, (size_t)c->k * c->LD * 8));
    HIPCHK(c, hipMemcpyAsync(c->Wprev, c->W, (size_t)c->k * c->ldw * 8, hipMemcpyDeviceToDevice, c->stream));
    HIPCHK(c, hipMemcpyAsync(c->Tprev, c->T, (size_t)c->k * c->LD * 8, hipMemcpyDeviceToDevice, c->stream));
    return RRI_OK;
}

rri_status rri_rollback(rri_ctx* c) {
    CHECK_CTX(c);
    if (!c->Wprev || !c->Tprev) return fail(c, RRI_ERR_INVALID, "no snapshot taken");
    HIPCHK(c, hipSetDevice(c->device));
    HIPCHK(c, hipMemcpyAsync(c->W, c->Wprev, (size_t)c->k * c->ldw * 8, hipMemcpyDeviceToDevice, c->stream));
    HIPCHK(c, hipMemcpyAsync(c->T, c->Tprev, (size_t)c->k * c->LD * 8, hipMemcpyDeviceToDevice, c->stream));
    HIPCHK(c, hipStreamSynchronize(c->stream));
    invalidate(c);
    c->q_valid = false; c->gfull_valid = false;
    c->pending_wcheck = false;
    return RRI_OK;
}

rri_status rri_residual_rebuild(rri_ctx* c) {
    CHECK_CTX(c);
    REFUSE_F16(c, "the explicit residual");
    if (!c->explicit_resid) return fail(c, RRI_ERR_INVALID, "handle was not created with RRI_UNWEIGHTED_RESIDUAL");
    if (!c->have_X || !c->have_W || !c->have_T) return fail(c, RRI_ERR_INVALID, "X, W, T must be set");
    HIPCHK(c, hipSetDevice(c->device));
    r_refresh(c);
    HIPCHK(c, hipStreamSynchronize(c->stream));
    return RRI_OK;
}

rri_status rri_get_residual(rri_ctx* c, void* host, int64_t ld, int32_t host_dtype) {
    CHECK_CTX(c);
    REFUSE_F16(c, "the explicit residual");
    if (!c->explicit_resid) return fail(c, RRI_ERR_INVALID, "handle was not created with RRI_UNWEIGHTED_RESIDUAL");
    HIPCHK(c, hipSetDevice(c->device));
    return to_host(c, c->E, c->LD, host, ld, host_dtype, c->n, c->d, c->dtype);
}

rri_status rri_residual_update(rri_ctx* c, const double* a, const double* b, const double* a2, const double* b2,
                               const double* trow, const double* wcol, double* y_out, double* z_out) {
    CHECK_CTX(c);
    REFUSE_F16(c, "the explicit residual");
    if (!c->explicit_resid) return fail(c, RRI_ERR_INVALID, "handle was not created with RRI_UNWEIGHTED_RESIDUAL");
    if (!a || !b || !trow || !wcol || ((a2 == nullptr) != (b2 == nullptr)))
        return fail(c, RRI_ERR_INVALID, "a, b, trow, wcol are required; a2 and b2 come together");
    HIPCHK(c, hipSetDevice(c->device));
    HIPCHK(c, clear_halt(c) == RRI_OK ? hipSuccess : hipErrorUnknown);
    DevTmp rows, cols;
    HIPCHK(c, rows.alloc((size_t)3 * c->n * sizeof(double)));
    HIPCHK(c, cols.alloc((size_t)3 * c->LD * sizeof(double)));
    double* dr = (double*)rows.p;
    double* dc = (double*)cols.p;
    HIPCHK(c, hipMemsetAsync(dc, 0, (size_t)3 * c->LD * sizeof(double), c->stream));
    const double* hr[3] = {a, a2, wcol};
    const double* hc[3] = {b, b2, trow};
    for (int q = 0; q < 3; ++q) {
        if (hr[q]) HIPCHK(c, hipMemcpyAsync(dr + (i64)q * c->n, hr[q], (size_t)c->n * sizeof(double), hipMemcpyHostToDevice, c->stream));
        if (hc[q]) HIPCHK(c, hipMemcpyAsync(dc + (i64)q * c->LD, hc[q], (size_t)c->d * sizeof(double), hipMemcpyHostToDevice, c->stream));
    }
    DISPATCH(c, {
        typename L::Upd u;
        u.a = dr;
        u.b = dc;
        if (a2) { u.a2 = dr + c->n; u.b2 = dc + c->LD; u.b2sub = c->zeros; }
        L::rank_update(c, c->E, c->LD, u, dc + 2 * c->LD, dr + 2 * c->n);
    });
    const int nb = (int)((c->LD + 31) / 32);
    hipLaunchKernelGGL(k_reduce, dim3(nb), dim3(1024), 0, c->stream, (const double*)c->Zpart, c->LD, c->nrb,
// ... 261 lines not shown
    REFUSE_F16(c, "preprocessing of the resident X (it ends in a rewrite of X, a second rounding: preprocess on the host)");
    if (!df_out) return fail(c, RRI_ERR_INVALID, "df_out is NULL");
    if (c->weighted || !c->have_X || c->sparse_x) return fail(c, RRI_ERR_INVALID, "needs an unweighted handle with a dense X");
    HIPCHK(c, hipSetDevice(c->device));
    HIPCHK(c, clear_halt(c) == RRI_OK ? hipSuccess : hipErrorUnknown);
    const int ncols = (int)std::min<i64>(c->ldx, c->LD);
    HIPCHK(c, hipMemsetAsync(c->Zpart, 0, (size_t)c->nrb * c->LD * sizeof(double), c->stream));
    DISPATCH(c, hipLaunchKernelGGL((k_col_count<typename L::Elem>), dim3(c->npanels * c->nrb), dim3(256), 0, c->stream,
                                   (const typename L::Elem*)c->X, c->ldx, (int)c->n, ncols, c->Zpart, c->LD, c->rpb,
                                   c->npanels));
    LK::reduce(c);
    HIPCHK(c, hipMemcpyAsync(df_out, c->red, (size_t)c->d * sizeof(double), hipMemcpyDeviceToHost, c->stream));
    HIPCHK(c, hipStreamSynchronize(c->stream));
    invalidate(c);
    return RRI_OK;
}

rri_status rri_scale_X(rri_ctx* c, const double* col_scale, int32_t normalize_rows) {
    CHECK_CTX(c);
    REFUSE_F16(c, "rewriting X in place (a second rounding: preprocess on the host, X is then rounded once at upload)");
    if (c->weighted || !c->have_X || c->sparse_x) return fail(c, RRI_ERR_INVALID, "needs an unweighted handle with a dense X");
    if (!c->own_X) return fail(c, RRI_ERR_INVALID, "X is bound caller memory: it is not rewritten in place");
    HIPCHK(c, hipSetDevice(c->device));
    HIPCHK(c, clear_halt(c) == RRI_OK ? hipSuccess : hipErrorUnknown);
    DevTmp sd, inv;
    double* sdev = nullptr;
    HIPCHK(c, sd.alloc((size_t)c->LD * sizeof(double)));
    sdev = (double*)sd.p;
    if (col_scale) {
        HIPCHK(c, hipMemsetAsync(sdev, 0, (size_t)c->LD * sizeof(double), c->stream));
        HIPCHK(c, hipMemcpyAsync(sdev, col_scale, (size_t)c->d * sizeof(double), hipMemcpyHostToDevice, c->stream));
    } else {
        std::vector<double> ones((size_t)c->LD, 0.0);
        std::fill(ones.begin(), ones.begin() + c->d, 1.0);
        HIPCHK(c, hipMemcpyAsync(sdev, ones.data(), (size_t)c->LD * sizeof(double), hipMemcpyHostToDevice, c->stream));
        HIPCHK(c, hipStreamSynchronize(c->stream));
    }
    double* invdev = nullptr;
    if (normalize_rows) {
        HIPCHK(c, inv.alloc((size_t)c->n * sizeof(double)));
        invdev = (double*)inv.p;
        const int tsave = c->timing;
        c->timing = 0;
        DISPATCH(c, (L::template pass_cfg<true, false, 0>(c, c->X, c->ldx, sdev, c->W, L::stream_whole(c))));
        c->timing = tsave;
        hipLaunchKernelGGL(k_row_inverse, dim3((unsigned)((c->n + 255) / 256)), dim3(256), 0, c->stream,
                           (const double*)c->Ypart, c->npanels, (int)c->n, invdev);
    }
    DISPATCH(c, hipLaunchKernelGGL((k_scale2d<typename L::Elem>), dim3(8192), dim3(256), 0, c->stream,
                                   (typename L::Elem*)c->X, c->ldx, c->n, (int)c->d, col_scale ? (const double*)sdev : nullptr,
                                   (const double*)invdev));
    HIPCHK(c, hipStreamSynchronize(c->stream));
    invalidate(c);
    c->q_valid = false; c->gfull_valid = false;
    c->x_sq_valid = false;
    return RRI_OK;
}

rri_status rri_csr_column_positive_counts(rri_ctx* c, double* df_out) {
    CHECK_CTX(c);
    if (!df_out) return fail(c, RRI_ERR_INVALID, "df_out is NULL");
    if (!c->sparse_x || !c->have_X) return fail(c, RRI_ERR_INVALID, "needs an RRI_UNWEIGHTED_SPARSE handle with an X");
    HIPCHK(c, hipSetDevice(c->device));
    DevTmp out;
    HIPCHK(c, out.alloc((size_t)c->d * sizeof(double)));
    const rri_ctx::SpCopy& cc = c->sp[1];
    DISPATCH(c, hipLaunchKernelGGL((k_spx_poscount<typename L::Elem>), dim3((unsigned)((c->d + 3) / 4)), dim3(256), 0, c->stream,
                                   (const i64*)cc.segptr, cc.nseg, cc.nblk, (const typename L::Elem*)cc.val, (double*)out.p));
    HIPCHK(c, hipMemcpyAsync(df_out, out.p, (size_t)c->d * sizeof(double), hipMemcpyDeviceToHost, c->stream));
    HIPCHK(c, hipStreamSynchronize(c->stream));
    return RRI_OK;
}

extern "C++" {
template <typename SX, int LPS>
static void launch_spx_scale_lps(rri_ctx* c, const double* sdev, double* tot, unsigned long long* nzero, bool totals) {
    const unsigned nb = (unsigned)((c->n + 256 / LPS - 1) / (256 / LPS));
    if (totals)
        hipLaunchKernelGGL((k_spx_rowtot<SX, LPS>), dim3(nb), dim3(256), 0, c->stream, (const i64*)c->sp_rowptr,
                           (const int*)c->sp_col, (const SX*)c->sp_x, c->n, sdev, tot, nzero);
    else
        hipLaunchKernelGGL((k_spx_scale<SX, LPS>), dim3(nb), dim3(256), 0, c->stream, (const i64*)c->sp_rowptr,
                           (const int*)c->sp_col, (SX*)c->sp_x, c->n, sdev, (const double*)tot);
}
template <typename SX>
static void launch_spx_scale(rri_ctx* c, const double* sdev, double* tot, unsigned long long* nzero, bool totals) {
    if (c->nnz / std::max<i64>(c->n, 1) >= 64) launch_spx_scale_lps<SX, 64>(c, sdev, tot, nzero, totals);
    else launch_spx_scale_lps<SX, 8>(c, sdev, tot, nzero, totals);
}
}

rri_status rri_csr_scale_X(rri_ctx* c, const double* col_scale, int32_t normalize_rows, int64_t* zero_rows_out) {
    CHECK_CTX(c);
    if (!c->sparse_x || !c->have_X) return fail(c, RRI_ERR_INVALID, "needs an RRI_UNWEIGHTED_SPARSE handle with an X");
    if (zero_rows_out) *zero_rows_out = 0;
    if (!col_scale && !normalize_rows) return RRI_OK;
    HIPCHK(c, hipSetDevice(c->device));
    HIPCHK(c, clear_halt(c) == RRI_OK ? hipSuccess : hipErrorUnknown);
    DevTmp sd, tt, nz;
    if (col_scale) {
        HIPCHK(c, sd.alloc((size_t)c->d * sizeof(double)));
        HIPCHK(c, hipMemcpyAsync(sd.p, col_scale, (size_t)c->d * sizeof(double), hipMemcpyHostToDevice, c->stream));
    }
    if (normalize_rows) {
        HIPCHK(c, tt.alloc((size_t)c->n * sizeof(double)));
        HIPCHK(c, nz.alloc(sizeof(unsigned long long)));
        HIPCHK(c, hipMemsetAsync(nz.p, 0, sizeof(unsigned long long), c->stream));
        DISPATCH(c, launch_spx_scale<typename L::Elem>(c, (const double*)sd.p, (double*)tt.p, (unsigned long long*)nz.p, true));
        unsigned long long zero_rows = 0;
        HIPCHK(c, hipMemcpyAsync(&zero_rows, nz.p, sizeof(zero_rows), hipMemcpyDeviceToHost, c->stream));
        HIPCHK(c, hipStreamSynchronize(c->stream));
        if (zero_rows > 0) {
            if (!zero_rows_out) return fail(c, RRI_ERR_INVALID, "%llu rows sum to less than 1e-10 and zero_rows_out is NULL", zero_rows);
            *zero_rows_out = (int64_t)zero_rows;
            return RRI_OK;
        }
    }
    DISPATCH(c, launch_spx_scale<typename L::Elem>(c, (const double*)sd.p, (double*)tt.p, nullptr, false));
    if (c->nnz > 0)
        DISPATCH(c, for (int w = 0; w < 2; ++w)
                        hipLaunchKernelGGL((k_sp_permute<typename L::Elem>), dim3(2048), dim3(256), 0, c->stream,
                                           (const typename L::Elem*)c->sp_x, (const int*)c->sp[w].perm, c->sp[w].count,
                                           (typename L::Elem*)c->sp[w].val));
    HIPCHK(c, hipStreamSynchronize(c->stream));
    invalidate(c);
    c->q_valid = false; c->gfull_valid = false;
    c->x_sq_valid = false;
    return RRI_OK;
}

rri_status rri_reduce_buffer(rri_ctx* c, void** dev_ptr, int64_t* n_elems) {
    CHECK_CTX(c);
    if (dev_ptr) *dev_ptr = (void*)c->red;
    if (n_elems) *n_elems = c->red_elems;
    return RRI_OK;
}

rri_status rri_bind_reduce_buffer(rri_ctx* c, void* dev_ptr, int64_t n_elems) {
    CHECK_CTX(c);
    if (!dev_ptr || n_elems < c->red_elems || ((uintptr_t)dev_ptr) % 16)
        return fail(c, RRI_ERR_INVALID, "reduce buffer needs >= %lld elements, 16-byte aligned", c->red_elems);
    if (c->own_red && c->red) (void)hipFree(c->red);
    c->red = (double*)dev_ptr;
    c->own_red = false;
    invalidate(c);
    return RRI_OK;
}

rri_status rri_topic_reduce_local(rri_ctx* c, int32_t t) {
    CHECK_CTX(c);
    rri_status r = ready(c);
    if (r != RRI_OK) return r;
    if (c->prm.fix_T) return fail(c, RRI_ERR_UNSUPPORTED, "split stepping is the T-row step taken apart: T must be free");
    if (c->explicit_resid) return fail(c, RRI_ERR_UNSUPPORTED, "row-sharded stepping runs the Gram-form schedule only");
    if (c->comm) return fail(c, RRI_ERR_INVALID, "a communicator is attached: rri_sweep does the collectives itself");
    if (t < 0 || t >= c->k) return fail(c, RRI_ERR_INVALID, "topic out of range");
    HIPCHK(c, hipSetDevice(c->device));
    if (c->weighted) {
        if (!c->resid_valid || (t == 0 && !c->resid_fresh)) w_refresh(c);
        enqueue_wT_sums(c, t);
        if (c->pending_wcheck)
            hipLaunchKernelGGL(k_wcheck_wcol, dim3(1), dim3(256), 0, c->stream, (const double*)c->Gpart, c->nwb256, c->k,
                               c->pending_wcheck_topic, 0, t, kparams(c), c->st, c->red + 2 * c->LD);
        else
            HIPCHK(c, hipMemsetAsync(c->red + 2 * c->LD, 0, 2 * sizeof(double), c->stream));
        return RRI_OK;
    }
    if (!c->carry_valid || c->carry_topic != t) {
        const bool pend = c->pending_wcheck;
        const int pt = c->pending_wcheck_topic;
        c->pending_wcheck = false;
        enqueue_prologue(c, t, 0);
        c->pending_wcheck = pend;
        c->pending_wcheck_topic = pt;
        if (pend) return fail(c, RRI_ERR_INVALID, "carry lost while a sharded column check was pending");
    }
    LK::reduce(c);
    return RRI_OK;
}
// ... 199 lines not shown
    DevTmp buf;
    HIPCHK(c, buf.alloc((size_t)count * sizeof(double)));
    HIPCHK(c, hipMemcpyAsync(buf.p, host, (size_t)count * 8, hipMemcpyHostToDevice, c->stream));
    comm_broadcast(c, (double*)buf.p, count, root);
    HIPCHK(c, hipMemcpyAsync(host, buf.p, (size_t)count * 8, hipMemcpyDeviceToHost, c->stream));
    HIPCHK(c, hipStreamSynchronize(c->stream));
    if (c->comm_status != RRI_OK) { const rri_status r = c->comm_status; c->comm_status = RRI_OK; return r; }
    return RRI_OK;
}

rri_status rri_comm_allreduce_sum(rri_ctx* c, double* host, int64_t count) {
    CHECK_CTX(c);
    if (!host || count < 1) return fail(c, RRI_ERR_INVALID, "bad all-reduce arguments");
    HIPCHK(c, hipSetDevice(c->device));
    if (count <= 8 || !c->comm) return comm_allreduce_host(c, host, count);
    DevTmp buf;
    HIPCHK(c, buf.alloc((size_t)count * sizeof(double)));
    HIPCHK(c, hipMemcpyAsync(buf.p, host, (size_t)count * 8, hipMemcpyHostToDevice, c->stream));
    comm_allreduce(c, (double*)buf.p, count);
    HIPCHK(c, hipMemcpyAsync(host, buf.p, (size_t)count * 8, hipMemcpyDeviceToHost, c->stream));
    HIPCHK(c, hipStreamSynchronize(c->stream));
    if (c->comm_status != RRI_OK) { const rri_status r = c->comm_status; c->comm_status = RRI_OK; return r; }
    return RRI_OK;
}

rri_status rri_comm_stats(rri_ctx* c, int32_t* rank, int32_t* world, int64_t* allreduce_calls) {
    CHECK_CTX(c);
    if (rank) *rank = c->comm ? c->comm->rank : 0;
    if (world) *world = c->comm ? c->comm->world : 1;
    if (allreduce_calls) *allreduce_calls = c->comm ? c->comm->n_allreduce : 0;
    return RRI_OK;
}

rri_status rri_onchip_info(rri_ctx* c, int32_t* eligible, int64_t* launches) {
    CHECK_CTX(c);
    if (eligible) *eligible = (c->have_X && c->have_params && onchip_ok(c)) ? 1 : 0;
    if (launches) *launches = c->onchip_launches;
    return RRI_OK;
}

rri_status rri_layout_info(rri_ctx* c, int64_t* out, int32_t n) {
    CHECK_CTX(c);
    if (!out || n < 1) return fail(c, RRI_ERR_INVALID, "rri_layout_info needs room for at least one value");
    const bool dense_w = c->weighted == RRI_WEIGHTED_DENSE;
    const int64_t v[RRI_LAYOUT_FIELDS] = {
        c->sparse ? c->sp[0].nblk : 0, c->sparse ? c->sp[0].bw : 0, c->sparse ? c->sp[0].lps : 0, c->sparse ? c->sp[0].nwork : 0,
        c->sparse ? c->sp[1].nblk : 0, c->sparse ? c->sp[1].bw : 0, c->sparse ? c->sp[1].lps : 0, c->sparse ? c->sp[1].nwork : 0,
        c->rpb, c->nrb, c->npanels,
        c->Mbits ? 1 : 0, c->Mcols ? 1 : 0,
        c->mcols_tried && c->Mbits ? (int64_t)(c->mask_density * 1.0e9 + 0.5) : -1,
        dense_w && wtrow_small(c) ? 1 : 0,
        dense_w && c->nw_mask ? 1 : 0,
        !c->sparse && ro_pass_interleaved(c) ? 1 : 0,
        c->wcorr_nrb, c->n_cu};
    for (int i = 0; i < n && i < RRI_LAYOUT_FIELDS; ++i) out[i] = v[i];
    return RRI_OK;
}

rri_status rri_debug_xcc(rri_ctx* c, int32_t* out, int32_t count) {
    CHECK_CTX(c);
    if (!out || count < 1 || count > 4096) return fail(c, RRI_ERR_INVALID, "bad count");
    HIPCHK(c, hipSetDevice(c->device));
    DevTmp dv;
    HIPCHK(c, dv.alloc((size_t)count * sizeof(int)));
    hipLaunchKernelGGL(k_xcc_probe, dim3((unsigned)count), dim3(64), 0, c->stream, (int*)dv.p);
    HIPCHK(c, hipMemcpyAsync(out, dv.p, (size_t)count * sizeof(int), hipMemcpyDeviceToHost, c->stream));
    HIPCHK(c, hipStreamSynchronize(c->stream));
    return RRI_OK;
}

rri_status rri_onchip_fallbacks(rri_ctx* c, int64_t* fallbacks) {
    CHECK_CTX(c);
    if (fallbacks) *fallbacks = c->onchip_fallbacks;
    return RRI_OK;
}

rri_status rri_timing_enable(rri_ctx* c, int32_t on) {
    CHECK_CTX(c);
    c->timing = on < 0 ? 0 : on;
    for (int i = 0; i < 4; ++i) c->timing_seq[i] = 0;
    return RRI_OK;
}

rri_status rri_timing_read(rri_ctx* c, int32_t id, int64_t* launches, double* total_ms) {
    CHECK_CTX(c);
    if (id < 0 || id > 3) return fail(c, RRI_ERR_INVALID, "kernel_id out of range");
    HIPCHK(c, hipSetDevice(c->device));
    HIPCHK(c, hipStreamSynchronize(c->stream));
    double tot = 0.0;
    for (auto& tl : c->timed[id]) {
        float ms = 0.f;
        HIPCHK(c, hipEventElapsedTime(&ms, tl.a, tl.b));
        tot += ms;
        c->event_pool.push_back(tl.a);
        c->event_pool.push_back(tl.b);
    }
    if (launches) *launches = (int64_t)c->timed[id].size();
    if (total_ms) *total_ms = tot;
    c->timed[id].clear();
    return RRI_OK;
}

rri_status rri_synchronize(rri_ctx* c) {
    CHECK_CTX(c);
    HIPCHK(c, hipSetDevice(c->device));
    HIPCHK(c, hipStreamSynchronize(c->stream));
    return RRI_OK;
// ... 73 lines not shown
```

### rri_nmf_amd/csrc/rri_kernels.hpp

```cpp
#pragma once
#include <type_traits>

#include "rri_device.hpp"
#include "rri_hip.h"

namespace rri {

enum { HALT_EVENT_RESET_T = 1, HALT_EVENT_RESET_W = 2,
       HALT_EVENT_STOP = 3,
       HALT_ERR_UNBOUNDED = -4, HALT_ERR_W_COL_ZERO = -5, HALT_ERR_NOT_IMPLEMENTED = -6 };
enum { RESET_NONE = 0, RESET_MAX_RESID = 1, RESET_RANDOM = 2 };

struct DevState {
    int halt;
    int halt_topic;
    int halt_sweep;
    int halt_pos;
    int tmode;
    int proj_iters;
    int pad0;
    int pad1;
    double nt1;
    double nt;
    double sumT;
// ... 15 lines not shown
    static constexpr int N = 4;
    static __device__ __forceinline__ void unpack(const f32x4& v, double (&o)[4]) {
        o[0] = (double)v[0]; o[1] = (double)v[1]; o[2] = (double)v[2]; o[3] = (double)v[3];
    }
    static __device__ __forceinline__ f32x4 pack(const double (&o)[4]) {
        return f32x4{(float)o[0], (float)o[1], (float)o[2], (float)o[3]};
    }
    static __device__ __forceinline__ f32x4 zero() { return f32x4{0.f, 0.f, 0.f, 0.f}; }
};
template <> struct XVec<double> {
    typedef f64x2 type;
    static constexpr int N = 2;
    static __device__ __forceinline__ void unpack(const f64x2& v, double (&o)[2]) { o[0] = v[0]; o[1] = v[1]; }
    static __device__ __forceinline__ f64x2 pack(const double (&o)[2]) { return f64x2{o[0], o[1]}; }
    static __device__ __forceinline__ f64x2 zero() { return f64x2{0.0, 0.0}; }
};
typedef _Float16 f16x8 __attribute__((ext_vector_type(8)));
typedef _Float16 f16x4 __attribute__((ext_vector_type(4)));
template <> struct XVec<_Float16> {
    typedef f16x8 type;
    static constexpr int N = 8;
    static __device__ __forceinline__ void unpack(const f16x8& v, double (&o)[8]) {
#pragma unroll
        for (int e = 0; e < 8; ++e) o[e] = (double)(float)v[e];
    }
    static __device__ __forceinline__ f16x8 pack(const double (&o)[8]) {
        f16x8 r;
#pragma unroll
        for (int e = 0; e < 8; ++e) r[e] = (_Float16)(float)o[e];
        return r;
    }
    static __device__ __forceinline__ f16x8 zero() {
        return f16x8{(_Float16)0.f, (_Float16)0.f, (_Float16)0.f, (_Float16)0.f, (_Float16)0.f, (_Float16)0.f, (_Float16)0.f, (_Float16)0.f};
    }
};

template <bool NT, typename V>
__device__ __forceinline__ V stream_load(const V* p) {
    if constexpr (NT) return __builtin_nontemporal_load(p);
    else return *p;
}

template <bool NT, typename V>
__device__ __forceinline__ void stream_store(V* p, const V& v) {
    if constexpr (NT) __builtin_nontemporal_store(v, p);
    else *p = v;
}

struct TgramJob {
    const double* T; i64 ldt; int d, k, t;
    double* Ttpart; const double* tpart; int ntb, nsplit, finish, sweep;
    KParams p; DevState* st;
    int nblocks;
};
__device__ __forceinline__ void tgram_block(const double* __restrict__ T, i64 ldt, int d, int k, int t, int l, int split,
                                            int ns, double* __restrict__ Ttpart, const double* __restrict__ tpart,
                                            int nblk, int finish, int sweep, const KParams& p, DevState* st,
                                            double* scratch) {
    const int chunk = (d + ns - 1) / ns;
    const int j0 = split * chunk, j1 = min(d, j0 + chunk);
    double acc = 0.0;
    for (int j = j0 + threadIdx.x; j < j1; j += 256) acc = fma(T[(i64)l * ldt + j], T[(i64)t * ldt + j], acc);
    acc = block_sum(acc, scratch);
    if (threadIdx.x == 0) Ttpart[split * k + l] = acc;
    if (finish && l == 0 && split == 0) {
        double ps = 0.0;
        ps = ordered_sum<4>(tpart, 1, threadIdx.x, nblk, 256);
        ps = block_sum(ps, scratch);
        if (threadIdx.x == 0) {
            const int mode = st->tmode;
            st->nt1 = (mode == 0) ? ps : 1.0;
            st->sumT = ps;
            if (!(ps > 1e-10) && p.reset_method != RESET_NONE && p.resets_left > 0) {
                st->halt = HALT_EVENT_RESET_T; st->halt_topic = t; st->halt_sweep = sweep; st->halt_pos = t;
            }
        }
    }
}

#define RRI_PASS_ROWS(LNT) \
    for (int l0 = 0; l0 < rpb; l0 += U) {                                                                         \
        const int r = grow(l0);                                        \
        if (r >= n) break;                                               \
        V x[U];                                                                                                   \
        _Pragma("unroll")                                                                                         \
        for (int u = 0; u < U; ++u) {                                                                             \
            const int rr = r + u;                                                                                 \
            x[u] = XV::zero();                                                                                    \
            if (rr < n && ok) x[u] = stream_load<LNT>(reinterpret_cast<const V*>(X + (i64)rr * ldx + col));       \
        }                                                                                                         \
        _Pragma("unroll")                                                                                         \
        for (int u = 0; u < U; ++u) {                                                                             \
            const int rr = r + u;                                                                                 \
            double wv = 0.0, na = 0.0, na2 = 0.0;                                                                 \
            if (DO_Z && rr < n) wv = wsh[l0 + u];                                                                 \
            if (UPD > 0 && rr < n) na = -ash[l0 + u];                                                             \
            if (UPD > 1 && rr < n) na2 = -ash2[l0 + u];                                                           \
            double xe[VN];                                                                                        \
            XV::unpack(x[u], xe);                                                                                 \
            if constexpr (UPD > 0) {                                                                              \
        _Pragma("unroll")                                                                                         \
                for (int e = 0; e < VN; ++e) {                                                                    \
                    xe[e] = fma(na, bv[e], xe[e]);                                                                \
                    if (UPD > 1) xe[e] = fma(na2, bv2[e], xe[e]);                                                 \
                }                                                                                                 \
                const V rounded = XV::pack(xe);                                                                   \
                if (rr < n && ok) stream_store<NT>(reinterpret_cast<V*>(X + (i64)rr * ldx + col), rounded);       \
                             \
                if constexpr (sizeof(SX) == 4) XV::unpack(rounded, xe);                                           \
            }                                                                                                     \
            double yp = 0.0;                                                                                      \
        _Pragma("unroll")                                                                                         \
            for (int e = 0; e < VN; ++e) {                                                                        \
                if (DO_Y) yp = fma(xe[e], tv[e], yp);                                                             \
                if (DO_Z) zacc[e] = fma(wv, xe[e], zacc[e]);                                                      \
            }                                                                                                     \
            if constexpr (DO_Y && RS) wave_rowsum8_park(tile, u, lane, yp);                                       \
            else if (DO_Y) {                                                                                      \
                 \
                const double tot = wave_sum_lane63<double>(yp);                                                   \
                if (lane == 63) ysh[wave * rpb + l0 + u] = tot;                                                   \
            }                                                                                                     \
        }                                                                                                         \
        if constexpr (DO_Y && RS) {                                                                               \
            const double tot = wave_rowsum8_finish(tile, lane);                                                   \
            if ((lane & 7) == 0) ysh[wave * rpb + l0 + (lane >> 3)] = tot;                                        \
        }                                                                                                         \
    }

template <typename SX, bool DO_Y, bool DO_Z, int UPD, int U, bool NT, bool RS>
__global__ __launch_bounds__(256) void k_pass(typename std::conditional<(UPD > 0), SX, const SX>::type* __restrict__ X,
                                              i64 ldx, int n, int ncols,
                                              const double* __restrict__ trow, const double* __restrict__ wcol,
                                              double* __restrict__ Ypart, double* __restrict__ Zpart, i64 ldz,
                                              int rpb, int npg, const double* __restrict__ avec,
                                              const double* __restrict__ bvec, const double* __restrict__ avec2,
                                              const double* __restrict__ bvec2, const double* __restrict__ bsub2,
                                              const DevState* __restrict__ st, const TgramJob job, int nrb_il_rot,
                                              int keep_q) {
    typedef XVec<SX> XV;
    typedef typename XV::type V;
    constexpr int VN = XV::N;
    constexpr int PW = 64 * VN;
    if (st->halt) return;
    if ((int)blockIdx.x < job.nblocks) {
        __shared__ double jscratch[40];
        tgram_block(job.T, job.ldt, job.d, job.k, job.t, (int)blockIdx.x % job.k, (int)blockIdx.x / job.k, job.nsplit,
                    job.Ttpart, job.tpart, job.ntb, job.finish, job.sweep, job.p, job.st, jscratch);
        return;
    }
    const int nrb_il = nrb_il_rot & 0x07ffffff;
    const int rot = (int)((unsigned)nrb_il_rot >> 27);
    int bid = (int)blockIdx.x - job.nblocks;
    if (rot != 0 && (bid | 7) < (int)gridDim.x - job.nblocks) bid = (bid & ~7) | ((bid + rot) & 7);
    extern __shared__ __attribute__((aligned(16))) unsigned char smem[];
    double* ysh = reinterpret_cast<double*>(smem);
    double* wsh = ysh + 4 * rpb;
    double* ash = wsh + rpb;
    double* ash2 = ash + rpb;
    static_assert(!RS || U == 8, "the LDS row-sum path reduces 8 rows at a time");
    const int lane = threadIdx.x & 63;
    const int wave = __builtin_amdgcn_readfirstlane(threadIdx.x >> 6);
    double* tile = wsh + (1 + UPD) * rpb + wave * (8 * 72);
    const int pg = bid % npg;
    const int rb = bid / npg;
    auto grow = [&](int li) -> int {
        return nrb_il > 0 ? ((li / U) * nrb_il + rb) * U + (li % U) : rb * rpb + li;
    };
    const int col = (pg * 4 + wave) * PW + lane * VN;
    if (DO_Z || UPD > 0) {
        for (int i = threadIdx.x; i < rpb; i += 256) {
            const int g = grow(i);
            if (DO_Z) wsh[i] = g < n ? wcol[g] : 0.0;
            if (UPD > 0) ash[i] = g < n ? avec[g] : 0.0;
            if (UPD > 1) ash2[i] = g < n ? avec2[g] : 0.0;
        }
        __syncthreads();
    }
    const bool ok = col < ncols;
    const bool wave_has_cols = (pg * 4 + wave) * PW < ncols;
    double tv[VN], zacc[VN], bv[VN], bv2[VN];
#pragma unroll
    for (int e = 0; e < VN; ++e) {
        zacc[e] = 0.0;
        tv[e] = (DO_Y && ok) ? trow[col + e] : 0.0;
        bv[e] = (UPD > 0 && ok) ? bvec[col + e] : 0.0;
        bv2[e] = (UPD > 1 && ok) ? bvec2[col + e] - bsub2[col + e] : 0.0;
    }
    if (wave_has_cols) {
        if constexpr (NT && UPD == 0) {
            const unsigned nrb = ((unsigned)gridDim.x - (unsigned)job.nblocks) / (unsigned)npg;
            const bool kept = ((unsigned)(rb + 1) * (unsigned)keep_q) / nrb != ((unsigned)rb * (unsigned)keep_q) / nrb;
            if (kept) { RRI_PASS_ROWS(false) }
            else { RRI_PASS_ROWS(true) }
        } else {
            RRI_PASS_ROWS(NT)
        }
        if (DO_Z && ok) {
#pragma unroll
            for (int e = 0; e < VN; ++e) Zpart[(i64)rb * ldz + col + e] = zacc[e];
        }
    } else if (DO_Y) {
        for (int i = lane; i < rpb; i += 64) ysh[wave * rpb + i] = 0.0;
    }
    if (DO_Y) {
        __syncthreads();
        for (int i = threadIdx.x; i < rpb; i += 256) {
            const int g = grow(i);
            if (g < n) Ypart[(i64)pg * n + g] = (ysh[i] + ysh[rpb + i]) + (ysh[2 * rpb + i] + ysh[3 * rpb + i]);
        }
    }
}

#undef RRI_PASS_ROWS

template <typename SX, int NV>
__global__ __launch_bounds__(256) void k_colsums(const SX* __restrict__ X, i64 ldx, int n, int ncols,
                                                 const double* __restrict__ Qt, i64 ldq, int nv,
                                                 double* __restrict__ Zmulti, i64 ldz, int rpb, int npg, int nrb) {
    typedef XVec<SX> XV;
    typedef typename XV::type V;
    constexpr int VN = XV::N;
    constexpr int PW = 64 * VN;
    constexpr int U = 4;
    extern __shared__ __attribute__((aligned(16))) unsigned char smem[];
    double* wsh = reinterpret_cast<double*>(smem);
    const int lane = threadIdx.x & 63;
    const int wave = __builtin_amdgcn_readfirstlane(threadIdx.x >> 6);
    const int pg = blockIdx.x % npg, rb = blockIdx.x / npg;
    const int row0 = rb * rpb, row1 = min(n, row0 + rpb);
    const int col = (pg * 4 + wave) * PW + lane * VN;
    for (int i = threadIdx.x; i < (row1 - row0) * NV; i += 256) {
        const int v = i / (row1 - row0), r = i - v * (row1 - row0);
        wsh[v * rpb + r] = v < nv ? Qt[(i64)v * ldq + row0 + r] : 0.0;
    }
    __syncthreads();
    if ((pg * 4 + wave) * PW >= ncols) return;
    const bool ok = col < ncols;
    double acc[NV][VN];
#pragma unroll
    for (int v = 0; v < NV; ++v)
#pragma unroll
        for (int e = 0; e < VN; ++e) acc[v][e] = 0.0;
    for (int r = row0; r < row1; r += U) {
// ... 140 lines not shown
        for (int l0 = wave; l0 < k; l0 += 4 * CH) {
            double wl[CH];
#pragma unroll
            for (int q = 0; q < CH; ++q) {
                const int l = l0 + 4 * q;
                wl[q] = (l < k && valid && !(UPDATE && l == t)) ? Wt[(i64)l * ldw + i] : 0.0;
            }
#pragma unroll
            for (int q = 0; q < CH; ++q) {
                const int l = l0 + 4 * q;
                if (l < k) {
                    if (UPDATE) dotv = fma(wl[q], tts[l], dotv);
                    if (CARRY && !(UPDATE && l == t)) {
                        const double g = wave_sum<double>(wn * wl[q]);
                        if (lane == 0) gsh[l] += g;
                    }
                }
            }
        }
        double wnew = 0.0;
        if (UPDATE) {
            dsh[wave * 64 + lane] = dotv;
            __syncthreads();
            if (wave == 0) {
                const double dot = (dsh[lane] + dsh[64 + lane]) + (dsh[128 + lane] + dsh[192 + lane]);
                if (valid) {
                    const double numer = (y - dot) - p.reg_w_l1;
                    if (mode == 0) wnew = fmax(numer, 0.0) / (cden + p.eps);
                    else wnew = (-numer + cden < 0.0) ? p.w_row_sum : 0.0;
                    Wt[(i64)t * ldw + i] = wnew;
                }
                wsh[lane] = wnew;
            }
            __syncthreads();
            wnew = wsh[lane];
        }
        if (wave == 0) {
            const double nwp = wave_sum<double>(wn * wn);
            const double swp = wave_sum<double>(wnew);
            if (lane == 0) { gsh[k] += nwp; gsh[k + 1] += swp; }
            if (UPDATE) {
                const double xy = wave_sum<double>(wnew * y);
                if (lane == 0) xyp[(i64)blockIdx.x * TILES + tile] = xy;
            }
        } else if (wave == 1 && UPDATE && CARRY) {
            const double gt = wave_sum<double>(wn * wnew);
            if (lane == 0) gsh[t] += gt;
        }
        if (UPDATE) __syncthreads();
    }
    __syncthreads();
    double* gp = Gpart + (i64)blockIdx.x * (k + 2);
    for (int l = tid; l < k + 2; l += 256) gp[l] = gsh[l];
}

__host__ __device__ constexpr int wsweep_kp(int k) { return (k + 3) & ~3; }
__host__ __device__ constexpr size_t wsweep_lds_bytes(int k) { return ((size_t)k * wsweep_kp(k) + 64 * (size_t)k) * sizeof(double); }

__global__ __launch_bounds__(64) void k_wsweep_rows(double* __restrict__ Wt, double* __restrict__ Wprev, i64 ldw, int n, int k,
                                                    int t0, const double* __restrict__ Qt, const double* __restrict__ G,
                                                    double* __restrict__ colsum, int nwb, double* __restrict__ xyp,
                                                    i64 xy_stride, KParams p, const DevState* __restrict__ st) {
    if (st->halt) return;
    extern __shared__ __attribute__((aligned(16))) unsigned char smem[];
    const int kp = wsweep_kp(k);
    double* gsh = reinterpret_cast<double*>(smem);
    double* wsh = gsh + (size_t)k * kp;
    const int lane = threadIdx.x;
    const i64 i = (i64)blockIdx.x * 64 + lane;
    const bool valid = i < n;
    for (int q = lane; q < k * kp; q += 64) {
        const int l = q / kp, c = q - l * kp;
        gsh[q] = c < k ? G[(i64)l * k + c] : 0.0;
    }
    constexpr int CH = 8;
    for (int l0 = 0; l0 < k; l0 += CH) {
        double wv[CH];
#pragma unroll
        for (int q = 0; q < CH; ++q) wv[q] = (l0 + q < k && valid) ? Wt[(i64)(l0 + q) * ldw + i] : 0.0;
#pragma unroll
        for (int q = 0; q < CH; ++q) {
            const int l = l0 + q;
            if (l < k) {
                wsh[l * 64 + lane] = wv[q];
                if (valid) Wprev[(i64)l * ldw + i] = wv[q];
            }
        }
    }
    const int tb0 = t0 & ~3;
    double yv[4], yn[4];
#pragma unroll
    for (int j = 0; j < 4; ++j) yv[j] = (tb0 + j < k && valid) ? Qt[(i64)(tb0 + j) * ldw + i] : 0.0;
    __syncthreads();
    for (int tb = tb0; tb < k; tb += 4) {
#pragma unroll
        for (int j = 0; j < 4; ++j) yn[j] = (tb + 4 + j < k && valid) ? Qt[(i64)(tb + 4 + j) * ldw + i] : 0.0;
        double acc[4] = {0.0, 0.0, 0.0, 0.0};
        auto outside = [&](int la, int lb) {
#pragma unroll 4
            for (int l = la; l < lb; ++l) {
                const double wl = wsh[l * 64 + lane];
                const f64x2 g01 = *reinterpret_cast<const f64x2*>(gsh + (size_t)l * kp + tb);
                const f64x2 g23 = *reinterpret_cast<const f64x2*>(gsh + (size_t)l * kp + tb + 2);
                acc[0] = fma(wl, g01[0], acc[0]);
                acc[1] = fma(wl, g01[1], acc[1]);
                acc[2] = fma(wl, g23[0], acc[2]);
// ... 137 lines not shown
__global__ __launch_bounds__(1024) void k_reduce(const double* __restrict__ Zpart, i64 ldz, int nrb,
                                                 const double* __restrict__ Gpart, int nwb, int k,
                                                 double* __restrict__ red, const DevState* __restrict__ st) {
    if (st->halt) return;
    __shared__ double sh[32 * 33];
    const int tid = threadIdx.x;
    const int ngram = Gpart ? GRAM_SLICES : 0;
    const int nzb = gridDim.x - ngram;
    if ((int)blockIdx.x < nzb) {
        const int c = tid & 31, g = tid >> 5;
        const i64 j = (i64)blockIdx.x * 32 + c;
        double a = 0.0;
        if (j < ldz) a = ordered_sum<8>(Zpart + j, ldz, g, nrb, 32);
        sh[g * 33 + c] = a;
        __syncthreads();
        if (tid < 32 && j < ldz) {
            double s = 0.0;
            for (int q = 0; q < 32; ++q) s += sh[q * 33 + tid];
            red[j] = s;
        }
    } else {
        const int gs = blockIdx.x - nzb;
        const int per = (nwb + GRAM_SLICES - 1) / GRAM_SLICES;
        const int b0 = gs * per, b1 = min(nwb, b0 + per);
        const int lane = tid & 63, wave = tid >> 6;
        for (int l0 = 0; l0 < k + 2; l0 += 64) {
            const int l = l0 + lane;
            double a = 0.0;
            if (l < k + 2) a = ordered_sum<8>(Gpart + l, k + 2, b0 + wave, b1, 16);
            __syncthreads();
            sh[wave * 64 + lane] = a;
            __syncthreads();
            if (wave == 0 && l < k + 2) {
                double s = 0.0;
                for (int q = 0; q < 16; ++q) s += sh[q * 64 + lane];
                red[ldz + (i64)gs * (k + 2) + l] = s;
            }
        }
    }
}

__device__ __forceinline__ double red_gram(const double* __restrict__ red, i64 ldz, int k, int l) {
    double s = 0.0;
#pragma unroll
    for (int g = 0; g < GRAM_SLICES; ++g) s += red[ldz + (i64)g * (k + 2) + l];
    return s;
}

__global__ __launch_bounds__(128) void k_trow_numer(double* __restrict__ T, i64 ldt, int d, int k, int t,
                                                    const double* __restrict__ red, i64 ldz,
                                                    double* __restrict__ xraw, double* __restrict__ tpart,
                                                    i64* __restrict__ tpart_idx, int check_prev, int tprev,
                                                    int sweep, KParams p, DevState* st, int resid_form,
                                                    double* __restrict__ told) {
    if (st->halt) return;
    const int tid = threadIdx.x;
    __shared__ double scratch[40];
    __shared__ double gsh[RRI_MAX_K];
    const double nw = red_gram(red, ldz, k, k);
    if (check_prev) {
        const double sw = red_gram(red, ldz, k, k + 1);
        const bool ev = (sw <= 1e-10) && p.reset_method != RESET_NONE && p.resets_left > 0;
        const bool err = !ev && !(sw > 0.0);
        if (ev || err) {
            if (blockIdx.x == 0 && tid == 0) {
                st->halt = ev ? HALT_EVENT_RESET_W : HALT_ERR_W_COL_ZERO;
                st->halt_topic = tprev; st->halt_sweep = sweep; st->halt_pos = t;
            }
            return;
        }
    }
    const double c = nw + p.reg_t_l2;
    const bool project = p.project_T && p.has_trs;
    int mode = 0;
    if (!(c > 0.0)) {
        if (!project) {
            if (p.has_trs && p.t_row_sum != 0.0) mode = 1;
            else mode = HALT_ERR_UNBOUNDED;
        } else {
            mode = (p.t_row_sum == 1.0) ? 2 : HALT_ERR_NOT_IMPLEMENTED;
        }
        if (mode < 0) {
            if (blockIdx.x == 0 && tid == 0) {
                st->halt = mode; st->halt_topic = t; st->halt_sweep = sweep; st->halt_pos = t;
            }
            return;
        }
    }
    for (int l = tid; l < k; l += 128) gsh[l] = (l == t) ? (resid_form ? -nw : 0.0) : red_gram(red, ldz, k, l);
    __syncthreads();
    const i64 j = (i64)blockIdx.x * 128 + tid;
    double x = 0.0, mx = -1.0e300;
    if (j < d) {
        if (told) told[j] = T[(i64)t * ldt + j];
        double a0 = 0.0, a1 = 0.0, a2 = 0.0, a3 = 0.0;
        for (int l0 = 0; l0 < k; l0 += 16) {
            double tv[16];
#pragma unroll
            for (int q = 0; q < 16; ++q) tv[q] = (l0 + q < k) ? T[(i64)(l0 + q) * ldt + j] : 0.0;
#pragma unroll
            for (int q = 0; q < 16; q += 4) {
                if (l0 + q < k) a0 = fma(gsh[l0 + q], tv[q], a0);
                if (l0 + q + 1 < k) a1 = fma(gsh[l0 + q + 1], tv[q + 1], a1);
                if (l0 + q + 2 < k) a2 = fma(gsh[l0 + q + 2], tv[q + 2], a2);
                if (l0 + q + 3 < k) a3 = fma(gsh[l0 + q + 3], tv[q + 3], a3);
            }
        }
        const double acc = (a0 + a1) + (a2 + a3);
        const double numer = (red[j] - acc) - p.reg_t_l1;
        if (mode == 0) x = fmax(numer, 0.0) / (c + p.eps);
        else if (mode == 1) x = (-numer + c < 0.0) ? p.t_row_sum : 0.0;
        else { x = numer; mx = numer; }
        xraw[j] = x;
        if (mode == 1 || (mode == 0 && !project)) T[(i64)t * ldt + j] = x;
    }
    if (mode != 2) {
        const double s = block_sum(x, scratch);
        if (tid == 0) tpart[blockIdx.x] = s;
    } else {
        i64 idx = (j < d) ? j : (i64)0x7fffffffffffffffLL;
        wave_argmax(mx, idx);
        __shared__ double wm[2];
        __shared__ i64 wi[2];
        if ((tid & 63) == 0) { wm[tid >> 6] = mx; wi[tid >> 6] = idx; }
        __syncthreads();
        if (tid == 0) {
            if (wm[1] > wm[0] || (wm[1] == wm[0] && wi[1] < wi[0])) { wm[0] = wm[1]; wi[0] = wi[1]; }
            tpart[blockIdx.x] = wm[0];
            tpart_idx[blockIdx.x] = wi[0];
        }
    }
    if (blockIdx.x == 0 && tid == 0) st->tmode = mode;
}

__global__ __launch_bounds__(1024) void k_trow_small(double* __restrict__ T, i64 ldt, int d, int k, int t,
                                                     const double* __restrict__ Zpart, int nrb,
                                                     const double* __restrict__ Gpart, int nwb, double* __restrict__ red,
                                                     i64 ldz, double* __restrict__ xraw, double* __restrict__ tpart,
                                                     i64* __restrict__ tpart_idx, int check_prev, int tprev, int sweep,
                                                     KParams p, DevState* st, int resid_form, double* __restrict__ told) {
    if (st->halt) return;
    const int tid = threadIdx.x;
    __shared__ double sh[32 * 33];
    __shared__ double gsh[RRI_MAX_K + 2];
    __shared__ double zs[32];
    const int cc = tid & 31, g = tid >> 5;
    const i64 j = (i64)blockIdx.x * 32 + cc;
    constexpr int ZB = 16;
    double zpre[ZB];
#pragma unroll
    for (int q = 0; q < ZB; ++q) {
        const int r = g + 32 * q;
        zpre[q] = (j < ldz && r < nrb) ? Zpart[(i64)r * ldz + j] : 0.0;
    }
    double tkeep[4];
#pragma unroll
    for (int q = 0; q < 4; ++q) {
        const int l = g + 32 * q;
        tkeep[q] = (j < d && l < k && (l != t || resid_form)) ? T[(i64)l * ldt + j] : 0.0;
    }
    for (int l0 = 0; l0 < k + 2; l0 += 32) {
        const int l = l0 + cc;
        double a = 0.0;
        if (l < k + 2) a = ordered_sum<8>(Gpart + l, k + 2, g, nwb, 32);
        __syncthreads();
        sh[g * 33 + cc] = a;
        __syncthreads();
        if (tid < 32 && l < k + 2) {
            double s = 0.0;
            for (int q = 0; q < 32; ++q) s += sh[q * 33 + tid];
            gsh[l] = s;
        }
    }
    __syncthreads();
    const double nw = gsh[k];
    if (check_prev) {
        const double sw = gsh[k + 1];
        const bool ev = (sw <= 1e-10) && p.reset_method != RESET_NONE && p.resets_left > 0;
        const bool err = !ev && !(sw > 0.0);
        if (ev || err) {
            if (blockIdx.x == 0 && tid == 0) {
                st->halt = ev ? HALT_EVENT_RESET_W : HALT_ERR_W_COL_ZERO;
                st->halt_topic = tprev; st->halt_sweep = sweep; st->halt_pos = t;
            }
            return;
// ... 114 lines not shown
    bool row_dirty = false;
    if (mode == 2) {
        double bm = tpart[0];
        i64 bi = tpart_idx[0];
        for (int b = 1; b < nblk; ++b)
            if (tpart[b] > bm) { bm = tpart[b]; bi = tpart_idx[b]; }
        for (int j = tid; j < d; j += blockDim.x) xraw[j] = (j == bi) ? 1.0 : 0.0;
        row_dirty = true;
    } else {
        double ps = 0.0;
        ps = ordered_sum<4>(tpart, 1, tid, nblk, (int)blockDim.x);
        ps = block_sum(ps, scratch);
        if (mode == 0) nx = ps;
        sumT = ps;
        if (mode == 0 && project) {
            const double th = simplex_theta(xraw, d, p.t_row_sum, scratch, &iters);
            for (int j = tid; j < d; j += blockDim.x) xraw[j] = fmax(xraw[j] - th, 0.0);
            if (tid == 0) st->theta = th;
            row_dirty = true;
        }
    }
    if (row_dirty) {
        __syncthreads();
        sumT = 0.0;
        for (int j = tid; j < d; j += blockDim.x) sumT += xraw[j];
        sumT = block_sum(sumT, scratch);
    }
    bool event = false;
    if (sumT > 1e-10 || p.reset_method == RESET_NONE) {
        if (p.has_trs && p.t_row_sum != 0.0 && p.project_T && fabs(sumT - p.t_row_sum) > 1e-15) {
            int it2 = 0;
            const double th = simplex_theta(xraw, d, p.t_row_sum, scratch, &it2);
            for (int j = tid; j < d; j += blockDim.x) xraw[j] = fmax(xraw[j] - th, 0.0);
            iters += it2;
            row_dirty = true;
        }
    } else if (p.resets_left > 0) {
        event = true;
    }
    if (row_dirty) {
        __syncthreads();
        for (int j = tid; j < d; j += blockDim.x) T[(i64)t * ldt + j] = xraw[j];
    }
    if (tid == 0) {
        st->nt1 = nx;
        st->sumT = sumT;
        st->proj_iters = iters;
        if (event) { st->halt = HALT_EVENT_RESET_T; st->halt_topic = t; st->halt_sweep = sweep; st->halt_pos = t; }
    }
}

__global__ __launch_bounds__(256) void k_tgram(const double* __restrict__ T, i64 ldt, int d, int k, int t,
                                               double* __restrict__ Ttpart, const double* __restrict__ tpart,
                                               int nblk, int finish, int sweep, KParams p, DevState* st) {
    if (st->halt) return;
    __shared__ double scratch[40];
    tgram_block(T, ldt, d, k, t, blockIdx.x, blockIdx.y, gridDim.y, Ttpart, tpart, nblk, finish, sweep, p, st, scratch);
}

__global__ __launch_bounds__(256) void k_scale_wcol(double* Wt, i64 ldw, int n, int t, const DevState* st) {
    if (st->halt) return;
    const i64 i = (i64)blockIdx.x * blockDim.x + threadIdx.x;
    if (i < n) Wt[(i64)t * ldw + i] *= st->nt1;
}

__global__ __launch_bounds__(64) void k_check_red(const double* __restrict__ red, i64 ldz, int k, int tprev,
                                                  int sweep, int pos, KParams p, DevState* st) {
    if (st->halt) return;
    if (threadIdx.x == 0) {
        const double sw = red_gram(red, ldz, k, k + 1);
        const bool ev = (sw <= 1e-10) && p.reset_method != RESET_NONE && p.resets_left > 0;
        const bool err = !ev && !(sw > 0.0);
        if (ev || err) {
            st->halt = ev ? HALT_EVENT_RESET_W : HALT_ERR_W_COL_ZERO;
            st->halt_topic = tprev; st->halt_sweep = sweep; st->halt_pos = pos;
        }
    }
}

__global__ __launch_bounds__(256) void k_check_wcol(const double* __restrict__ Gpart, int nwb, int k, int tprev,
                                                    int sweep, int pos, KParams p, DevState* st) {
    if (st->halt) return;
    __shared__ double scratch[40];
    double a = 0.0;
    a = ordered_sum<8>(Gpart + k + 1, k + 2, threadIdx.x, nwb, (int)blockDim.x);
    a = block_sum(a, scratch);
    if (threadIdx.x == 0) {
        const bool ev = (a <= 1e-10) && p.reset_method != RESET_NONE && p.resets_left > 0;
        const bool err = !ev && !(a > 0.0);
        if (ev || err) {
            st->halt = ev ? HALT_EVENT_RESET_W : HALT_ERR_W_COL_ZERO;
            st->halt_topic = tprev; st->halt_sweep = sweep; st->halt_pos = pos;
        }
    }
}

__global__ __launch_bounds__(256) void k_colsum_tail(const double* __restrict__ Gpart, int nwb, int k,
                                                     double* __restrict__ tail, const DevState* __restrict__ st) {
    if (st->halt) return;
    __shared__ double scratch[40];
    double a = ordered_sum<8>(Gpart + k + 1, k + 2, threadIdx.x, nwb, (int)blockDim.x);
    a = block_sum(a, scratch);
    if (threadIdx.x == 0) { tail[0] = a; tail[1] = 0.0; }
}

__global__ void k_pack_candidate(const double* __restrict__ rowpos, const i64* __restrict__ idx, i64 row_offset,
                                 double* __restrict__ out) {
    const i64 i = idx[0];
    out[0] = rowpos[i];
// ... 677 lines not shown
```

### rri_nmf_amd/engine.py

```python
import ctypes as C

import numpy as np

from . import _capi
from ._capi import Params, Event

EPS_DIV = float(np.spacing(10))

_NP2RRI = {np.dtype(np.float32): _capi.RRI_F32, np.dtype(np.float64): _capi.RRI_F64, np.dtype(np.float16): _capi.RRI_F16}
_HOST_TYPES = (np.dtype(np.float32), np.dtype(np.float64))
_RESET_CODES = {None: _capi.RESET_NONE, 'max_resid_document': _capi.RESET_MAX_RESID_DOCUMENT,
                'random': _capi.RESET_RANDOM}


class ZeroTotalRows(ValueError):

    def __init__(self, count):
        ValueError.__init__(self, '%d row(s) of X sum to less than 1e-10: normalisation would make them dense (1/d), which an X '
                                  'kept as CSR cannot hold; X was left unchanged' % count)
        self.count = int(count)


def _as_host(a, what, half=False):
    a = np.asarray(a)
# ... 535 lines not shown
            wR = r[:d] - wW.dot(self.get_T())
        return r, wR, nw, None

    def topic_sums(self, t):
        ld = -(-self.d // (16 // self.dtype.itemsize)) * (16 // self.dtype.itemsize)
        self.topic_reduce_local(t)
        _, wR, nw, _ = self._topic_sums(t, ld)
        return np.array(wR), (np.array(nw) if self.weighted else nw)

    def topic_finish_w(self, t):
        self._check(self._lib.rri_topic_finish_w(self._h, int(t)))

    def poll(self):
        return self._check(self._lib.rri_poll(self._h))

    def pending_event(self):
        ev = Event()
        self._check(self._lib.rri_pending_event(self._h, C.byref(ev)))
        return ev.kind, ev.topic, ev.resume_topic

    def resid_row_argmax(self):
        val, row = C.c_double(0.0), C.c_int64(-1)
        self._check(self._lib.rri_resid_row_argmax(self._h, C.byref(val), C.byref(row)))
        return float(val.value), int(row.value)

    def reset_row(self, local_row):
        out = np.empty(self.d, dtype=np.float64)
        self._check(self._lib.rri_reset_row(self._h, int(local_row), out.ctypes.data_as(C.POINTER(C.c_double))))
        return out

    def apply_reset_vectors(self, t, T_row, W_col):
        T_row = np.ascontiguousarray(T_row, dtype=np.float64)
        W_col = np.ascontiguousarray(W_col, dtype=np.float64)
        self._check(self._lib.rri_apply_reset_vectors(
            self._h, int(t), T_row.ctypes.data_as(C.POINTER(C.c_double)),
            W_col.ctypes.data_as(C.POINTER(C.c_double))))
        self.n_resets_used += 1

    def timing_enable(self, on=True, every=1):
        self._check(self._lib.rri_timing_enable(self._h, int(every) if on else 0))

    def timing_read(self, kernel_id):
        cnt, ms = C.c_int64(0), C.c_double(0.0)
        self._check(self._lib.rri_timing_read(self._h, int(kernel_id), C.byref(cnt), C.byref(ms)))
        return int(cnt.value), float(ms.value)

    def onchip_info(self):
        el, n = C.c_int32(0), C.c_int64(0)
        self._check(self._lib.rri_onchip_info(self._h, C.byref(el), C.byref(n)))
        return bool(el.value), int(n.value)

    LAYOUT_COPY_FIELDS = ('nblk', 'bw', 'lps', 'nwork')
    LAYOUT_FIELDS = ('rpb', 'nrb', 'npanels', 'mask_bits', 'mask_cols', 'mask_density', 'wtrow_small', 'nw_from_mask',
                     'interleaved', 'wcorr_nrb', 'n_cu')
    assert 2 * len(LAYOUT_COPY_FIELDS) + len(LAYOUT_FIELDS) == _capi.RRI_LAYOUT_FIELDS

    def layout_info(self):
        nc = len(self.LAYOUT_COPY_FIELDS)
        out = (C.c_int64 * _capi.RRI_LAYOUT_FIELDS)()
        self._check(self._lib.rri_layout_info(self._h, out, _capi.RRI_LAYOUT_FIELDS))
        v = [int(x) for x in out]
        info = {name: (v[i], v[nc + i]) for i, name in enumerate(self.LAYOUT_COPY_FIELDS)}
        info.update(zip(self.LAYOUT_FIELDS, v[2 * nc:]))
        for name in ('mask_bits', 'mask_cols', 'wtrow_small', 'nw_from_mask', 'interleaved'):
            info[name] = bool(info[name])
        info['mask_density'] = None if info['mask_density'] < 0 else info['mask_density'] * 1e-9
        return info

    def debug_xcc(self, count=32):
        out = (C.c_int32 * count)()
        self._check(self._lib.rri_debug_xcc(self._h, out, count))
        return list(out)

    def onchip_fallbacks(self):
        n = C.c_int64(0)
        self._check(self._lib.rri_onchip_fallbacks(self._h, C.byref(n)))
        return int(n.value)

    def sweep_until(self, n_sweeps, obj_prev, stop_scale):
        n_sweeps = int(n_sweeps)
        if not self.onchip_info()[0]:
            return None
        hist = np.full(n_sweeps, np.nan, dtype=np.float64)
        done = C.c_int32(0)
        st = self._lib.rri_sweep_until(self._h, n_sweeps, float(obj_prev), float(stop_scale),
                                       hist.ctypes.data_as(C.POINTER(C.c_double)), C.byref(done))
        if st == _capi.RRI_ERR_UNSUPPORTED:
            return None
        n_done = self._drive(st, done)
        return n_done, hist[:n_done]

    def synchronize(self):
        self._check(self._lib.rri_synchronize(self._h))

    def bench_rank1_update(self, reps=5):
        ms = C.c_double(0.0)
        self._check(self._lib.rri_bench_rank1_update(self._h, int(reps), C.byref(ms)))
        return float(ms.value)

    def bench_stream_copy(self, reps=5):
        ms = C.c_double(0.0)
        self._check(self._lib.rri_bench_stream_copy(self._h, int(reps), C.byref(ms)))
        return float(ms.value)
```

Measured before the change: 29.23.

## Fuse T-gram into trow kernel and split W-column update around the pass

The T-row numerator kernel now also writes the per-block partials of T·T_t, so the separate tgram launch can be skipped or reduced to a finish-only block. The W-column update is split: a pre-phase that computes the W·(TT) dot products runs as extra blocks inside the fused X pass, and a lightweight post kernel finishes the column. An occupancy hint (waves_per_eu) is also added to k_pass. The intent is fewer serialized launches and less duplicated work per topic, at the cost of extra register and shared-memory pressure in the trow kernel and more complex state tracking through tt_valid.

```diff
diff --git a/include/rri_hip.h b/include/rri_hip.h
--- a/include/rri_hip.h
+++ b/include/rri_hip.h
@@ -145,7 +145,7 @@
 rri_status rri_timing_read(rri_ctx* ctx, int32_t kernel_id, int64_t* launches, double* total_ms);
 rri_status rri_synchronize(rri_ctx* ctx);
 rri_status rri_onchip_info(rri_ctx* ctx, int32_t* eligible, int64_t* launches);
-#define RRI_LAYOUT_FIELDS 19
+#define RRI_LAYOUT_FIELDS 20
 rri_status rri_layout_info(rri_ctx* ctx, int64_t* out, int32_t n);
 rri_status rri_onchip_fallbacks(rri_ctx* ctx, int64_t* fallbacks);
 rri_status rri_debug_xcc(rri_ctx* ctx, int32_t* out, int32_t count);
diff --git a/rri_nmf_amd/_capi.py b/rri_nmf_amd/_capi.py
--- a/rri_nmf_amd/_capi.py
+++ b/rri_nmf_amd/_capi.py
@@ -5,7 +5,7 @@
 LIB_PATH = os.environ.get('RRI_HIP_LIB', os.path.join(_PKG, 'lib', 'librri_hip.so'))
 
 RRI_GRAM_SLICES = 8
-RRI_LAYOUT_FIELDS = 19
+RRI_LAYOUT_FIELDS = 20
 RRI_MAX_K = 1024
 RRI_OK, RRI_PAUSED = 0, 1
 RRI_ERR_INVALID, RRI_ERR_HIP, RRI_ERR_UNSUPPORTED = -1, -2, -3
diff --git a/rri_nmf_amd/csrc/rri_hip.hip b/rri_nmf_amd/csrc/rri_hip.hip
--- a/rri_nmf_amd/csrc/rri_hip.hip
+++ b/rri_nmf_amd/csrc/rri_hip.hip
@@ -115,6 +115,8 @@
     int rot_cal = 1;
     bool rot_debug = false;
     bool mask_bits = true;
+    bool wcol_split = true;
+    bool trow_small = true;
     double pass_cache_mb = PASS_CACHE_MB;
 };
 
@@ -192,6 +194,10 @@
     int npanels = 1, rpb = 1, nrb = 1, nwb = 1, ntb = 1;
     int gpart_n = 1;
     int ttpart_n = 0;
+    bool tt_valid = false;
+    int tt_topic = -1;
+    i64 wcol_splits = 0;
+    double* wdot = nullptr;
     int xy_rows = 0;
     int xy_stride = 1;
     int ntb32 = 1;
@@ -438,7 +444,7 @@
                        int keep) {
         const int ncols = (int)std::min<i64>(ldp, c->LD);
         typedef typename std::conditional<(UPD > 0), SX, const SX>::type XT;
-        hipLaunchKernelGGL((k_pass<SX, DO_Y, DO_Z, UPD, U, NT, RS>), dim3(c->npanels * c->nrb + job.nblocks), dim3(256),
+        hipLaunchKernelGGL((k_pass<SX, DO_Y, DO_Z, UPD, U, NT, RS>), dim3(c->npanels * c->nrb + job.nblocks + job.npre), dim3(256),
                            pass_shmem(c, UPD), c->stream, (XT*)Xp, ldp, (int)c->n, ncols, trow, wc, c->Ypart,
                            c->Zpart, c->LD, c->rpb, c->npanels, u.a, u.b, u.a2, u.b2, u.b2sub, (const DevState*)c->st, job,
                            ((ro_pass_interleaved(c) || UPD > 0) ? c->nrb : 0) |
@@ -913,10 +919,14 @@
     }
     static bool light(const rri_ctx* c) { return !(c->prm.project_T_each_iter && c->prm.has_t_row_sum); }
     static void trow(rri_ctx* c, int t, int check_prev, int tprev, int sweep, bool force_final) {
+        const bool tt = light(c) && !resid_sched(c);
         hipLaunchKernelGGL(k_trow_numer, dim3(c->ntb), dim3(128), 0, c->stream, c->T, c->LD, (int)c->d, c->k, t,
                            (const double*)c->red, c->LD, c->xraw, c->tpart, c->tpart_idx, check_prev, tprev, sweep,
-                           kparams(c), c->st, resid_sched(c) ? 1 : 0, resid_sched(c) ? c->told : (double*)nullptr);
+                           kparams(c), c->st, resid_sched(c) ? 1 : 0, resid_sched(c) ? c->told : (double*)nullptr,
+                           tt ? c->Ttpart : (double*)nullptr);
         c->tpart_n = c->ntb;
+        c->tt_valid = tt;
+        c->tt_topic = t;
         trow_final_if_needed(c, t, sweep, force_final);
     }
     static bool small(const rri_ctx* c) {
@@ -928,6 +938,7 @@
                            c->tpart, c->tpart_idx, check_prev, tprev, sweep, kparams(c), c->st, resid_sched(c) ? 1 : 0,
                            resid_sched(c) ? c->told : (double*)nullptr);
         c->tpart_n = c->ntb32;
+        c->tt_valid = false;
         trow_final_if_needed(c, t, sweep, force_final);
     }
     static void trow_final_if_needed(rri_ctx* c, int t, int sweep, bool force_final) {
@@ -941,9 +952,24 @@
     }
     static void tgram(rri_ctx* c, int t, int finish, int sweep) {
         c->ttpart_n = c->nsplit;
+        c->tt_valid = false;
         hipLaunchKernelGGL(k_tgram, dim3(c->k, c->nsplit), dim3(256), 0, c->stream, (const double*)c->T, c->LD,
                            (int)c->d, c->k, t, c->Ttpart, (const double*)c->tpart, c->tpart_n, finish, sweep,
-                           kparams(c), c->st);
+                           kparams(c), c->st, 0);
+    }
+    static void tgram_finish(rri_ctx* c, int t, int sweep) {
+        hipLaunchKernelGGL(k_tgram, dim3(1, 1), dim3(256), 0, c->stream, (const double*)c->T, c->LD,
+                           (int)c->d, c->k, t, c->Ttpart, (const double*)c->tpart, c->tpart_n, 1, sweep,
+                           kparams(c), c->st, 1);
+    }
+    static void wcol_post(rri_ctx* c, int t, int tn, int sweep) {
+        TimedScope ts(c, 1);
+        hipLaunchKernelGGL(k_wcol_post, dim3((c->nwb + 3) / 4), dim3(256), 0, c->stream, c->W, c->ldw, (int)c->n, c->k, t, tn,
+                           (const double*)c->Ypart, c->npanels, (const double*)c->wdot, c->Gpart,
+                           c->XYpart + (i64)t * c->xy_stride, sweep, kparams(c), c->st);
+        c->gpart_n = c->nwb;
+        c->wcol_splits += 1;
+        note_xy(c, t, c->nwb * WCOL_TILES);
     }
     static void scale_wcol(rri_ctx* c, int t) {
         hipLaunchKernelGGL(k_scale_wcol, dim3((unsigned)((c->n + 255) / 256)), dim3(256), 0, c->stream, c->W,
@@ -1092,6 +1118,7 @@
 
 void invalidate(rri_ctx* c) {
     c->carry_valid = false;
+    c->tt_valid = false;
     c->carry_topic = -1;
     c->resid_valid = false;
     c->xy_run = -1;
@@ -1134,7 +1161,7 @@
     {
         TimedScope ts(c, 2);
         const int chk = c->pending_wcheck ? 1 : 0;
-        if (LK::small(c) && !c->comm) {
+        if (LK::small(c) && !c->comm && c->sw.trow_small) {
             LK::trow_small(c, t, chk, c->pending_wcheck_topic, sweep, standalone);
         } else {
             LK::reduce(c);
@@ -1157,18 +1184,28 @@
     const int tn = (t + 1) % k;
     const int finish = (LK::light(c) && !c->prm.fix_T && !c->skip_row_finish) ? 1 : 0;
     c->skip_row_finish = false;
+    const bool tt = c->tt_valid && c->tt_topic == t && !c->prm.fix_T;
+    const bool split = tt && carry_next && LK::light(c) && c->sw.wcol_split && !c->sparse_x;
     TgramJob job{};
     if (c->prm.fix_T || c->sparse_x) {
         TimedScope ts(c, 2);
-        LK::tgram(c, t, finish, sweep);
+        if (!tt) LK::tgram(c, t, finish, sweep);
+        else if (finish) LK::tgram_finish(c, t, sweep);
     } else {
         job = TgramJob{(const double*)c->T, c->LD, (int)c->d, c->k, t, c->Ttpart, (const double*)c->tpart, c->tpart_n,
-                       c->nsplit, finish, sweep, kparams(c), c->st, c->k * c->nsplit};
-        c->ttpart_n = c->nsplit;
-    }
+                       c->nsplit, finish, sweep, kparams(c), c->st, tt ? finish : c->k * c->nsplit, tt ? 1 : 0};
+        if (!tt) { c->ttpart_n = c->nsplit; c->tt_valid = false; }
+        if (split) {
+            job.npre = (c->nwb + WPRE_TILES - 1) / WPRE_TILES;
+            job.n = (int)c->n; job.tn = tn; job.nparts = c->ntb;
+            job.Wt = c->W; job.ldw = c->ldw; job.Gpart = c->Gpart; job.wdot = c->wdot;
+        }
+    }
+    if (tt) c->ttpart_n = c->ntb;
     if (carry_next) {
         DISPATCH_RO(c, (L::template pass<true, true>(c, t, tn, job)));
-        LK::wcol<true, true>(c, t, tn, sweep);
+        if (split) LK::wcol_post(c, t, tn, sweep);
+        else LK::wcol<true, true>(c, t, tn, sweep);
         c->carry_valid = true;
         c->carry_topic = tn;
         c->pending_wcheck = true;
@@ -1216,7 +1253,7 @@
     {
         TimedScope ts(c, 2);
         const int chk = c->pending_wcheck ? 1 : 0;
-        if (LK::small(c) && !c->comm) {
+        if (LK::small(c) && !c->comm && c->sw.trow_small) {
             LK::trow_small(c, t, chk, c->pending_wcheck_topic, sweep, standalone);
         } else {
             LK::reduce(c);
@@ -1241,6 +1278,7 @@
     const TgramJob job{(const double*)c->T, c->LD, (int)c->d, c->k, t, c->Ttpart, (const double*)c->tpart, c->tpart_n,
                        c->nsplit, finish, sweep, kparams(c), c->st, c->k * c->nsplit};
     c->ttpart_n = c->nsplit;
+    c->tt_valid = false;
     const double* trow = c->T + (i64)t * c->LD;
     DISPATCH(c, {
         typename L::Upd u;
@@ -1752,7 +1790,7 @@
     const bool whole_last = c->run_total - 1 > cur.sweep || (cur.topic == 0 && cur.phase == 0);
     c->carry_valid = false; c->carry_topic = -1;
     c->pending_wcheck = false;
-    c->resid_valid = false; c->q_valid = false; c->gfull_valid = false;
+    c->resid_valid = false; c->q_valid = false; c->gfull_valid = false; c->tt_valid = false;
     c->skip_row_finish = false;
     c->xy_run = whole_last ? k : -1;
     c->xy_rows = g.G;
@@ -1857,6 +1895,8 @@
     if (const char* e = getenv("RRI_ROT_CAL")) sw.rot_cal = std::max(0, atoi(e));
     sw.rot_debug = getenv("RRI_ROT_DEBUG") != nullptr;
     if (const char* e = getenv("RRI_MASK_BITS")) sw.mask_bits = atoi(e) != 0;
+    if (const char* e = getenv("RRI_WCOL_SPLIT")) sw.wcol_split = atoi(e) != 0;
+    if (const char* e = getenv("RRI_TROW_SMALL")) sw.trow_small = atoi(e) != 0;
     if (const char* e = getenv("RRI_PASS_CACHE_MB")) sw.pass_cache_mb = std::max(0.0, atof(e));
     return sw;
 }
@@ -1998,11 +2038,13 @@
     c->own_red = true;
     CR(hipMalloc((void**)&c->xraw, (size_t)c->LD * f8));
     CR(hipMemsetAsync(c->xraw, 0, (size_t)c->LD * f8, c->stream));
-    const size_t ttn = (size_t)std::max(c->nsplit, c->ntb32);
+    const size_t ttn = (size_t)std::max(std::max(c->nsplit, c->ntb), c->ntb32);
     c->ttpart_n = c->nsplit;
     CR(hipMalloc((void**)&c->Ttpart, ttn * k * f8));
     CR(hipMemsetAsync(c->Ttpart, 0, ttn * k * f8, c->stream));
     CR(hipMalloc((void**)&c->Qt, (size_t)k * c->ldw * f8));
+    CR(hipMalloc((void**)&c->wdot, (size_t)(c->ldw + 8) * f8));
+    CR(hipMemsetAsync(c->wdot, 0, (size_t)(c->ldw + 8) * f8, c->stream));
     const size_t ntp = (size_t)std::max(c->ntb, c->ntb32);
     CR(hipMalloc((void**)&c->tpart, ntp * sizeof(double)));
     CR(hipMemsetAsync(c->tpart, 0, ntp * sizeof(double), c->stream));
@@ -2071,7 +2113,7 @@
     if (c->stream) (void)hipStreamSynchronize(c->stream);
     if (c->own_X) (void)hipFree(c->X);
     if (c->own_M) (void)hipFree(c->M);
-    void* bufs[] = {c->E, (void*)c->W, (void*)c->T, (void*)c->Wprev, (void*)c->Tprev,                     (void*)c->Ypart, (void*)c->Zpart, (void*)c->xraw, (void*)c->Ttpart, (void*)c->Gpart,
+    void* bufs[] = {c->E, (void*)c->W, (void*)c->T, (void*)c->Wprev, (void*)c->Tprev,                     (void*)c->Ypart, (void*)c->Zpart, (void*)c->xraw, (void*)c->Ttpart, (void*)c->wdot, (void*)c->Gpart,
                     (void*)c->tpart, (void*)c->tpart_idx, (void*)c->rowobj, (void*)c->rowpos, (void*)c->normpart,
                     (void*)c->dtmp, (void*)c->itmp, (void*)c->resetT, (void*)c->resetW, (void*)c->st, (void*)c->Y2part,
                     (void*)c->Z2part, (void*)c->Mbits, (void*)c->Qt, (void*)c->dtv, (void*)c->dwv, (void*)c->wold, (void*)c->zeros,
@@ -2102,7 +2144,7 @@
     c->ldx = c->LD;
     c->store_err[0] = c->store_err[1] = 0.0;
     rri_status s = to_device(c, host, ld, host_dtype, c->X, c->ldx, c->n, c->d, c->dtype);
-    if (s == RRI_OK || c->dtype == RRI_F16) { c->have_X = s == RRI_OK; invalidate(c); c->q_valid = false; c->gfull_valid = false; c->x_sq_valid = false; }
+    if (s == RRI_OK || c->dtype == RRI_F16) { c->have_X = s == RRI_OK; invalidate(c); c->q_valid = false; c->gfull_valid = false; c->tt_valid = false; c->x_sq_valid = false; }
     return s;
 }
 
@@ -2190,7 +2232,7 @@
     HIPCHK(c, hipStreamSynchronize(c->stream));
     c->have_X = true;
     invalidate(c);
-    c->q_valid = false; c->gfull_valid = false;
+    c->q_valid = false; c->gfull_valid = false; c->tt_valid = false;
     c->x_sq_valid = false;
     return RRI_OK;
 }
@@ -2251,7 +2293,7 @@
     HIPCHK(c, hipStreamSynchronize(c->stream));
     c->have_X = true;
     invalidate(c);
-    c->q_valid = false; c->gfull_valid = false;
+    c->q_valid = false; c->gfull_valid = false; c->tt_valid = false;
     c->x_sq_valid = false;
     return RRI_OK;
 }
@@ -2445,7 +2487,7 @@
     c->store_err[0] = c->store_err[1] = 0.0;
     c->have_X = true;
     invalidate(c);
-    c->q_valid = false; c->gfull_valid = false;
+    c->q_valid = false; c->gfull_valid = false; c->tt_valid = false;
     c->x_sq_valid = false;
     return RRI_OK;
 }
@@ -2483,7 +2525,7 @@
     CHECK_CTX(c);
     HIPCHK(c, hipSetDevice(c->device));
     rri_status s = to_device(c, host, ld, host_dtype, c->T, c->LD, c->k, c->d, RRI_F64);
-    if (s == RRI_OK) { c->have_T = true; invalidate(c); c->q_valid = false; c->gfull_valid = false; }
+    if (s == RRI_OK) { c->have_T = true; invalidate(c); c->q_valid = false; c->gfull_valid = false; c->tt_valid = false; }
     return s;
 }
 rri_status rri_get_W(rri_ctx* c, void* host, int64_t ld, int32_t host_dtype) {
@@ -2634,7 +2676,7 @@
 }
 
 static void event_resolved(rri_ctx* c) {
-    c->q_valid = false; c->gfull_valid = false;
+    c->q_valid = false; c->gfull_valid = false; c->tt_valid = false;
     if (c->pending.kind == RRI_EVENT_RESET_T) c->skip_row_finish = true;
     c->pending.kind = RRI_EVENT_NONE;
     if (c->prm.resets_left > 0) c->prm.resets_left -= 1;
@@ -3002,7 +3044,7 @@
     HIPCHK(c, hipMemcpyAsync(c->T, c->Tprev, (size_t)c->k * c->LD * 8, hipMemcpyDeviceToDevice, c->stream));
     HIPCHK(c, hipStreamSynchronize(c->stream));
     invalidate(c);
-    c->q_valid = false; c->gfull_valid = false;
+    c->q_valid = false; c->gfull_valid = false; c->tt_valid = false;
     c->pending_wcheck = false;
     return RRI_OK;
 }
@@ -3370,7 +3412,7 @@
                                    (const double*)invdev));
     HIPCHK(c, hipStreamSynchronize(c->stream));
     invalidate(c);
-    c->q_valid = false; c->gfull_valid = false;
+    c->q_valid = false; c->gfull_valid = false; c->tt_valid = false;
     c->x_sq_valid = false;
     return RRI_OK;
 }
@@ -3442,7 +3484,7 @@
                                            (typename L::Elem*)c->sp[w].val));
     HIPCHK(c, hipStreamSynchronize(c->stream));
     invalidate(c);
-    c->q_valid = false; c->gfull_valid = false;
+    c->q_valid = false; c->gfull_valid = false; c->tt_valid = false;
     c->x_sq_valid = false;
     return RRI_OK;
 }
@@ -3748,7 +3790,7 @@
         dense_w && wtrow_small(c) ? 1 : 0,
         dense_w && c->nw_mask ? 1 : 0,
         !c->sparse && ro_pass_interleaved(c) ? 1 : 0,
-        c->wcorr_nrb, c->n_cu};
+        c->wcorr_nrb, c->n_cu, c->wcol_splits};
     for (int i = 0; i < n && i < RRI_LAYOUT_FIELDS; ++i) out[i] = v[i];
     return RRI_OK;
 }
diff --git a/rri_nmf_amd/csrc/rri_kernels.hpp b/rri_nmf_amd/csrc/rri_kernels.hpp
--- a/rri_nmf_amd/csrc/rri_kernels.hpp
+++ b/rri_nmf_amd/csrc/rri_kernels.hpp
@@ -91,7 +91,26 @@
     double* Ttpart; const double* tpart; int ntb, nsplit, finish, sweep;
     KParams p; DevState* st;
     int nblocks;
+    int finish_only;
+    int npre;
+    int n, tn, nparts;
+    const double* Wt; i64 ldw;
+    double* Gpart; double* wdot;
 };
+__device__ __forceinline__ void trow_finish_block(const double* __restrict__ tpart, int nblk, int t, int sweep,
+                                                  const KParams& p, DevState* st, double* scratch) {
+    double ps = 0.0;
+    ps = ordered_sum<4>(tpart, 1, threadIdx.x, nblk, 256);
+    ps = block_sum(ps, scratch);
+    if (threadIdx.x == 0) {
+        const int mode = st->tmode;
+        st->nt1 = (mode == 0) ? ps : 1.0;
+        st->sumT = ps;
+        if (!(ps > 1e-10) && p.reset_method != RESET_NONE && p.resets_left > 0) {
+            st->halt = HALT_EVENT_RESET_T; st->halt_topic = t; st->halt_sweep = sweep; st->halt_pos = t;
+        }
+    }
+}
 __device__ __forceinline__ void tgram_block(const double* __restrict__ T, i64 ldt, int d, int k, int t, int l, int split,
                                             int ns, double* __restrict__ Ttpart, const double* __restrict__ tpart,
                                             int nblk, int finish, int sweep, const KParams& p, DevState* st,
@@ -102,18 +121,62 @@
     for (int j = j0 + threadIdx.x; j < j1; j += 256) acc = fma(T[(i64)l * ldt + j], T[(i64)t * ldt + j], acc);
     acc = block_sum(acc, scratch);
     if (threadIdx.x == 0) Ttpart[split * k + l] = acc;
-    if (finish && l == 0 && split == 0) {
-        double ps = 0.0;
-        ps = ordered_sum<4>(tpart, 1, threadIdx.x, nblk, 256);
-        ps = block_sum(ps, scratch);
-        if (threadIdx.x == 0) {
-            const int mode = st->tmode;
-            st->nt1 = (mode == 0) ? ps : 1.0;
-            st->sumT = ps;
-            if (!(ps > 1e-10) && p.reset_method != RESET_NONE && p.resets_left > 0) {
-                st->halt = HALT_EVENT_RESET_T; st->halt_topic = t; st->halt_sweep = sweep; st->halt_pos = t;
-            }
-        }
+    if (finish && l == 0 && split == 0) trow_finish_block(tpart, nblk, t, sweep, p, st, scratch);
+}
+
+constexpr int WPRE_TILES = 4;
+__device__ __forceinline__ void wcol_pre_block(const TgramJob& job, int jb, double* sm) {
+    const int tid = threadIdx.x, lane = tid & 63, wave = tid >> 6;
+    const int k = job.k, t = job.t, n = job.n;
+    const double* __restrict__ Wt = job.Wt;
+    const i64 ldw = job.ldw;
+    double* tts = sm;
+    double* dsh = sm + k;
+    for (int l = tid; l < k; l += 256) tts[l] = ordered_sum<8>(job.Ttpart + l, k, 0, job.nparts, 1);
+    __syncthreads();
+    if (jb == 0 && tid == 0) job.wdot[ldw] = tts[t];
+    __syncthreads();
+    if (tid == 0) tts[t] = 0.0;
+    __syncthreads();
+    constexpr int CH = 4;
+#pragma unroll 1
+    for (int q4 = 0; q4 < WPRE_TILES; ++q4) {
+        const i64 tile = (i64)jb * WPRE_TILES + q4;
+        if (tile * 64 >= n) break;
+        const i64 i = tile * 64 + lane;
+        const bool valid = i < n;
+        const double wn = valid ? Wt[(i64)job.tn * ldw + i] : 0.0;
+        double* gp = job.Gpart + tile * (k + 2);
+        double dotv = 0.0;
+#pragma unroll 1
+        for (int l0 = wave; l0 < k; l0 += 4 * CH) {
+            double wl[CH];
+#pragma unroll
+            for (int q = 0; q < CH; ++q) {
+                const int l = l0 + 4 * q;
+                wl[q] = (l < k && valid && l != t) ? Wt[(i64)l * ldw + i] : 0.0;
+            }
+#pragma unroll
+            for (int q = 0; q < CH; ++q) {
+                const int l = l0 + 4 * q;
+                if (l < k) {
+                    dotv = fma(wl[q], tts[l], dotv);
+                    if (l != t) {
+                        const double g = wave_sum<double>(wn * wl[q]);
+                        if (lane == 0) gp[l] = 0.0 + g;
+                    }
+                }
+            }
+        }
+        dsh[wave * 64 + lane] = dotv;
+        __syncthreads();
+        if (wave == 0) {
+            const double dot = (dsh[lane] + dsh[64 + lane]) + (dsh[128 + lane] + dsh[192 + lane]);
+            if (valid) job.wdot[i] = dot;
+            const double nwp = wave_sum<double>(wn * wn);
+            if (lane == 0) gp[k] = 0.0 + nwp;
+        }
+        __syncthreads();
     }
 }
 
@@ -167,8 +230,11 @@
         }                                                                                                         \
     }
 
+template <typename SX, bool DO_Y, bool DO_Z, int UPD>
+constexpr int pass_min_waves() { return (UPD == 0 && DO_Y && DO_Z) ? (sizeof(SX) == 8 ? 6 : sizeof(SX) == 4 ? 4 : 2) : 1; }
+
 template <typename SX, bool DO_Y, bool DO_Z, int UPD, int U, bool NT, bool RS>
-__global__ __launch_bounds__(256) void k_pass(typename std::conditional<(UPD > 0), SX, const SX>::type* __restrict__ X,
+__global__ __launch_bounds__(256) __attribute__((amdgpu_waves_per_eu(pass_min_waves<SX, DO_Y, DO_Z, UPD>()))) void k_pass(typename std::conditional<(UPD > 0), SX, const SX>::type* __restrict__ X,
                                               i64 ldx, int n, int ncols,
                                               const double* __restrict__ trow, const double* __restrict__ wcol,
                                               double* __restrict__ Ypart, double* __restrict__ Zpart, i64 ldz,
@@ -182,17 +248,25 @@
     constexpr int VN = XV::N;
     constexpr int PW = 64 * VN;
     if (st->halt) return;
+    extern __shared__ __attribute__((aligned(16))) unsigned char smem[];
+    const int npass = (int)gridDim.x - job.nblocks - job.npre;
     if ((int)blockIdx.x < job.nblocks) {
         __shared__ double jscratch[40];
-        tgram_block(job.T, job.ldt, job.d, job.k, job.t, (int)blockIdx.x % job.k, (int)blockIdx.x / job.k, job.nsplit,
-                    job.Ttpart, job.tpart, job.ntb, job.finish, job.sweep, job.p, job.st, jscratch);
+        if (job.finish_only) trow_finish_block(job.tpart, job.ntb, job.t, job.sweep, job.p, job.st, jscratch);
+        else tgram_block(job.T, job.ldt, job.d, job.k, job.t, (int)blockIdx.x % job.k, (int)blockIdx.x / job.k, job.nsplit,
+                         job.Ttpart, job.tpart, job.ntb, job.finish, job.sweep, job.p, job.st, jscratch);
         return;
+    }
+    if constexpr (DO_Y && DO_Z && UPD == 0) {
+        if ((int)blockIdx.x - job.nblocks >= npass) {
+            wcol_pre_block(job, (int)blockIdx.x - job.nblocks - npass, reinterpret_cast<double*>(smem));
+            return;
+        }
     }
     const int nrb_il = nrb_il_rot & 0x07ffffff;
     const int rot = (int)((unsigned)nrb_il_rot >> 27);
     int bid = (int)blockIdx.x - job.nblocks;
-    if (rot != 0 && (bid | 7) < (int)gridDim.x - job.nblocks) bid = (bid & ~7) | ((bid + rot) & 7);
-    extern __shared__ __attribute__((aligned(16))) unsigned char smem[];
+    if (rot != 0 && (bid | 7) < (int)gridDim.x - job.nblocks - job.npre) bid = (bid & ~7) | ((bid + rot) & 7);
     double* ysh = reinterpret_cast<double*>(smem);
     double* wsh = ysh + 4 * rpb;
     double* ash = wsh + rpb;
@@ -228,7 +302,7 @@
     }
     if (wave_has_cols) {
         if constexpr (NT && UPD == 0) {
-            const unsigned nrb = ((unsigned)gridDim.x - (unsigned)job.nblocks) / (unsigned)npg;
+            const unsigned nrb = ((unsigned)gridDim.x - (unsigned)job.nblocks - (unsigned)job.npre) / (unsigned)npg;
             const bool kept = ((unsigned)(rb + 1) * (unsigned)keep_q) / nrb != ((unsigned)rb * (unsigned)keep_q) / nrb;
             if (kept) { RRI_PASS_ROWS(false) }
             else { RRI_PASS_ROWS(true) }
@@ -475,6 +549,47 @@
     __syncthreads();
     double* gp = Gpart + (i64)blockIdx.x * (k + 2);
     for (int l = tid; l < k + 2; l += 256) gp[l] = gsh[l];
+}
+
+__global__ __launch_bounds__(256) void k_wcol_post(double* __restrict__ Wt, i64 ldw, int n, int k, int t, int tn,
+                                                   const double* __restrict__ Ypart, int npanels,
+                                                   const double* __restrict__ wdot, double* __restrict__ Gpart,
+                                                   double* __restrict__ xyp, int sweep, KParams p, DevState* st) {
+    if (st->halt) return;
+    const int tid = threadIdx.x, lane = tid & 63, wave = tid >> 6;
+    const double cden = wdot[ldw] + p.reg_w_l2;
+    int mode = 0;
+    if (!(cden > 0.0)) {
+        if (p.has_wrs && p.w_row_sum != 0.0) mode = 1;
+        else {
+            if (blockIdx.x == 0 && tid == 0) {
+                st->halt = HALT_ERR_UNBOUNDED; st->halt_topic = t; st->halt_sweep = sweep; st->halt_pos = t;
+            }
+            return;
+        }
+    }
+    const i64 tile = (i64)blockIdx.x * 4 + wave;
+    if (tile * 64 >= n) return;
+    const i64 i = tile * 64 + lane;
+    const bool valid = i < n;
+    const double wn = valid ? Wt[(i64)tn * ldw + i] : 0.0;
+    double y = 0.0, wnew = 0.0;
+    if (valid) {
+        y = ordered_sum<8>(Ypart + i, n, 0, npanels, 1);
+        const double numer = (y - wdot[i]) - p.reg_w_l1;
+        if (mode == 0) wnew = fmax(numer, 0.0) / (cden + p.eps);
+        else wnew = (-numer + cden < 0.0) ? p.w_row_sum : 0.0;
+        Wt[(i64)t * ldw + i] = wnew;
+    }
+    const double swp = wave_sum<double>(wnew);
+    const double xy = wave_sum<double>(wnew * y);
+    const double gt = wave_sum<double>(wn * wnew);
+    if (lane == 0) {
+        double* gp = Gpart + tile * (k + 2);
+        gp[t] = 0.0 + gt;
+        gp[k + 1] = 0.0 + swp;
+        xyp[tile] = xy;
+    }
 }
 
 __host__ __device__ constexpr int wsweep_kp(int k) { return (k + 3) & ~3; }
@@ -718,7 +833,7 @@
                                                     double* __restrict__ xraw, double* __restrict__ tpart,
                                                     i64* __restrict__ tpart_idx, int check_prev, int tprev,
                                                     int sweep, KParams p, DevState* st, int resid_form,
-                                                    double* __restrict__ told) {
+                                                    double* __restrict__ told, double* __restrict__ Ttp) {
     if (st->halt) return;
     const int tid = threadIdx.x;
     __shared__ double scratch[40];
@@ -797,6 +912,25 @@
         }
     }
     if (blockIdx.x == 0 && tid == 0) st->tmode = mode;
+    if (Ttp && (mode == 1 || (mode == 0 && !project))) {
+        __shared__ double psh[RRI_MAX_K];
+        __syncthreads();
+        double* mine = (tid >> 6) == 0 ? gsh : psh;
+        for (int l0 = 0; l0 < k; l0 += 16) {
+            double tv[16];
+#pragma unroll
+            for (int q = 0; q < 16; ++q) tv[q] = (l0 + q < k && l0 + q != t && j < d) ? T[(i64)(l0 + q) * ldt + j] : 0.0;
+#pragma unroll
+            for (int q = 0; q < 16; ++q) {
+                if (l0 + q < k) {
+                    const double s = wave_sum<double>((l0 + q == t ? x : tv[q]) * x);
+                    if ((tid & 63) == 0) mine[l0 + q] = s;
+                }
+            }
+        }
+        __syncthreads();
+        for (int l = tid; l < k; l += 128) Ttp[(i64)blockIdx.x * k + l] = gsh[l] + psh[l];
+    }
 }
 
 __global__ __launch_bounds__(1024) void k_trow_small(double* __restrict__ T, i64 ldt, int d, int k, int t,
@@ -1017,9 +1151,10 @@
 
 __global__ __launch_bounds__(256) void k_tgram(const double* __restrict__ T, i64 ldt, int d, int k, int t,
                                                double* __restrict__ Ttpart, const double* __restrict__ tpart,
-                                               int nblk, int finish, int sweep, KParams p, DevState* st) {
+                                               int nblk, int finish, int sweep, KParams p, DevState* st, int finish_only) {
     if (st->halt) return;
     __shared__ double scratch[40];
+    if (finish_only) { trow_finish_block(tpart, nblk, t, sweep, p, st, scratch); return; }
     tgram_block(T, ldt, d, k, t, blockIdx.x, blockIdx.y, gridDim.y, Ttpart, tpart, nblk, finish, sweep, p, st, scratch);
 }
 
diff --git a/rri_nmf_amd/engine.py b/rri_nmf_amd/engine.py
--- a/rri_nmf_amd/engine.py
+++ b/rri_nmf_amd/engine.py
@@ -611,7 +611,7 @@
 
     LAYOUT_COPY_FIELDS = ('nblk', 'bw', 'lps', 'nwork')
     LAYOUT_FIELDS = ('rpb', 'nrb', 'npanels', 'mask_bits', 'mask_cols', 'mask_density', 'wtrow_small', 'nw_from_mask',
-                     'interleaved', 'wcorr_nrb', 'n_cu')
+                     'interleaved', 'wcorr_nrb', 'n_cu', 'wcol_split')
     assert 2 * len(LAYOUT_COPY_FIELDS) + len(LAYOUT_FIELDS) == _capi.RRI_LAYOUT_FIELDS
 
     def layout_info(self):
```

After: 28.48. 2.6% lower.
